# ygina/sidekick

Measured on AMD Instinct MI355X. Metric: quACK encode identifiers/s (device-resident), u32 ids, threshold t=32, higher is better.
Workload: dtype u32; 1 GPU; encode 1e+09 u32 ids per GPU at t=32, device-resident; ids_per_gpu=1000000000, global_ids=1000000000, threshold=32, bits=32, seed=0x5eed0002, parallelism=shard1, collectives=single

## Files before the change

### sidekick_amd/csrc/bsgs.h

```cpp
#pragma once
#include <hip/hip_runtime.h>
#include <stdint.h>

#include "field.h"

namespace qk {
namespace bsgs {

constexpr int BLOCK = 256;
constexpr int WAVES = BLOCK / 64;

__device__ __forceinline__ uint64_t shfl_xor_u64(uint64_t v, int m) {
    const uint32_t lo = __shfl_xor((int)(uint32_t)v, m, 64);
    const uint32_t hi = __shfl_xor((int)(uint32_t)(v >> 32), m, 64);
    return ((uint64_t)hi << 32) | lo;
}

#define QK_MAC4V(P0, P1, P2, P3)                                                                       \
    "v_mad_u64_u32 %0, " P0 ", %8, %9, %0\n\t"                                                         \
    "v_mad_u64_u32 %1, " P1 ", %8, %10, %1\n\t"                                                        \
    "v_mad_u64_u32 %2, " P2 ", %8, %11, %2\n\t"                                                        \
    "v_mad_u64_u32 %3, " P3 ", %8, %12, %3\n\t"                                                        \
    "v_addc_co_u32_e64 %4, " P0 ", %4, 0, " P0 "\n\t"                                                  \
    "v_addc_co_u32_e64 %5, " P1 ", %5, 0, " P1 "\n\t"                                                  \
    "v_addc_co_u32_e64 %6, " P2 ", %6, 0, " P2 "\n\t"                                                  \
    "v_addc_co_u32_e64 %7, " P3 ", %7, 0, " P3
#define QK_MAC4S(P0, P1, P2, P3, T)                                                                       \
    "v_mad_u64_u32 %0, " P0 ", %8, %9, %0\n\t"                                                         \
    "v_mad_u64_u32 %1, " P1 ", %8, %10, %1\n\t"                                                        \
    "v_mad_u64_u32 %2, " P2 ", %8, %11, %2\n\t"                                                        \
    "v_mad_u64_u32 %3, " P3 ", %8, %12, %3\n\t"                                                        \
    "s_bcnt1_i32_b64 " T ", " P0 "\n\ts_add_u32 %4, %4, " T "\n\t"                                          \
    "s_bcnt1_i32_b64 " T ", " P1 "\n\ts_add_u32 %5, %5, " T "\n\t"                                          \
    "s_bcnt1_i32_b64 " T ", " P2 "\n\ts_add_u32 %6, %6, " T "\n\t"                                          \
    "s_bcnt1_i32_b64 " T ", " P3 "\n\ts_add_u32 %7, %7, " T
#define QK_ADD4V(P0, P1, P2, P3)                                                                       \
    "v_add_co_u32_e64 %0, " P0 ", %0, %8\n\t"                                                          \
    "v_add_co_u32_e64 %1, " P1 ", %1, %9\n\t"                                                          \
    "v_add_co_u32_e64 %2, " P2 ", %2, %10\n\t"                                                         \
    "v_add_co_u32_e64 %3, " P3 ", %3, %11\n\t"                                                         \
    "v_addc_co_u32_e64 %4, " P0 ", %4, 0, " P0 "\n\t"                                                  \
    "v_addc_co_u32_e64 %5, " P1 ", %5, 0, " P1 "\n\t"                                                  \
    "v_addc_co_u32_e64 %6, " P2 ", %6, 0, " P2 "\n\t"                                                  \
    "v_addc_co_u32_e64 %7, " P3 ", %7, 0, " P3
#define QK_ADD4S(P0, P1, P2, P3, T)                                                                       \
    "v_add_co_u32_e64 %0, " P0 ", %0, %8\n\t"                                                          \
    "v_add_co_u32_e64 %1, " P1 ", %1, %9\n\t"                                                          \
    "v_add_co_u32_e64 %2, " P2 ", %2, %10\n\t"                                                         \
    "v_add_co_u32_e64 %3, " P3 ", %3, %11\n\t"                                                         \
    "s_bcnt1_i32_b64 " T ", " P0 "\n\ts_add_u32 %4, %4, " T "\n\t"                                          \
    "s_bcnt1_i32_b64 " T ", " P1 "\n\ts_add_u32 %5, %5, " T "\n\t"                                          \
    "s_bcnt1_i32_b64 " T ", " P2 "\n\ts_add_u32 %6, %6, " T "\n\t"                                          \
    "s_bcnt1_i32_b64 " T ", " P3 "\n\ts_add_u32 %7, %7, " T
#define QK_SET0 "s[40:41]", "s[42:43]", "s[44:45]", "s[46:47]"
#define QK_SET1 "s[48:49]", "s[50:51]", "s[52:53]", "s[54:55]"
#define QK_SET0T QK_SET0, "s56"
#define QK_SET1T QK_SET1, "s57"
#define QK_CLOB0 "s40", "s41", "s42", "s43", "s44", "s45", "s46", "s47"
#define QK_CLOB1 "s48", "s49", "s50", "s51", "s52", "s53", "s54", "s55"
#define QK_EXPAND(M, ...) M(__VA_ARGS__)

template <int SET>
__device__ __forceinline__ void mac4v(uint64_t &a0, uint64_t &a1, uint64_t &a2, uint64_t &a3, uint32_t &c0,
                                      uint32_t &c1, uint32_t &c2, uint32_t &c3, uint32_t A, uint32_t b0,
                                      uint32_t b1, uint32_t b2, uint32_t b3) {
    if constexpr (SET == 0)
        asm volatile(QK_EXPAND(QK_MAC4V, QK_SET0)
            : "+v"(a0), "+v"(a1), "+v"(a2), "+v"(a3), "+v"(c0), "+v"(c1), "+v"(c2), "+v"(c3)
            : "v"(A), "v"(b0), "v"(b1), "v"(b2), "v"(b3)
            : QK_CLOB0);
    else
        asm volatile(QK_EXPAND(QK_MAC4V, QK_SET1)
            : "+v"(a0), "+v"(a1), "+v"(a2), "+v"(a3), "+v"(c0), "+v"(c1), "+v"(c2), "+v"(c3)
            : "v"(A), "v"(b0), "v"(b1), "v"(b2), "v"(b3)
            : QK_CLOB1);
}
template <int SET>
__device__ __forceinline__ void mac4s(uint64_t &a0, uint64_t &a1, uint64_t &a2, uint64_t &a3, uint32_t &s0,
                                      uint32_t &s1, uint32_t &s2, uint32_t &s3, uint32_t A, uint32_t b0,
                                      uint32_t b1, uint32_t b2, uint32_t b3) {
    if constexpr (SET == 0)
        asm volatile(QK_EXPAND(QK_MAC4S, QK_SET0T)
            : "+v"(a0), "+v"(a1), "+v"(a2), "+v"(a3), "+s"(s0), "+s"(s1), "+s"(s2), "+s"(s3)
            : "v"(A), "v"(b0), "v"(b1), "v"(b2), "v"(b3)
            : "scc", "s56", QK_CLOB0);
    else
        asm volatile(QK_EXPAND(QK_MAC4S, QK_SET1T)
            : "+v"(a0), "+v"(a1), "+v"(a2), "+v"(a3), "+s"(s0), "+s"(s1), "+s"(s2), "+s"(s3)
            : "v"(A), "v"(b0), "v"(b1), "v"(b2), "v"(b3)
            : "scc", "s57", QK_CLOB1);
}
template <int SET>
__device__ __forceinline__ void add4v(uint32_t &l0, uint32_t &l1, uint32_t &l2, uint32_t &l3, uint32_t &c0,
                                      uint32_t &c1, uint32_t &c2, uint32_t &c3, uint32_t b0, uint32_t b1,
                                      uint32_t b2, uint32_t b3) {
    if constexpr (SET == 0)
        asm volatile(QK_EXPAND(QK_ADD4V, QK_SET0)
            : "+v"(l0), "+v"(l1), "+v"(l2), "+v"(l3), "+v"(c0), "+v"(c1), "+v"(c2), "+v"(c3)
            : "v"(b0), "v"(b1), "v"(b2), "v"(b3)
            : QK_CLOB0);
    else
        asm volatile(QK_EXPAND(QK_ADD4V, QK_SET1)
            : "+v"(l0), "+v"(l1), "+v"(l2), "+v"(l3), "+v"(c0), "+v"(c1), "+v"(c2), "+v"(c3)
            : "v"(b0), "v"(b1), "v"(b2), "v"(b3)
            : QK_CLOB1);
}
template <int SET>
__device__ __forceinline__ void add4s(uint32_t &l0, uint32_t &l1, uint32_t &l2, uint32_t &l3, uint32_t &s0,
                                      uint32_t &s1, uint32_t &s2, uint32_t &s3, uint32_t b0, uint32_t b1,
                                      uint32_t b2, uint32_t b3) {
    if constexpr (SET == 0)
        asm volatile(QK_EXPAND(QK_ADD4S, QK_SET0T)
            : "+v"(l0), "+v"(l1), "+v"(l2), "+v"(l3), "+s"(s0), "+s"(s1), "+s"(s2), "+s"(s3)
            : "v"(b0), "v"(b1), "v"(b2), "v"(b3)
            : "scc", "s56", QK_CLOB0);
    else
        asm volatile(QK_EXPAND(QK_ADD4S, QK_SET1T)
            : "+v"(l0), "+v"(l1), "+v"(l2), "+v"(l3), "+s"(s0), "+s"(s1), "+s"(s2), "+s"(s3)
            : "v"(b0), "v"(b1), "v"(b2), "v"(b3)
            : "scc", "s57", QK_CLOB1);
}
__device__ __forceinline__ void mac2v(uint64_t &a0, uint64_t &a1, uint32_t &c0, uint32_t &c1, uint32_t A,
                                      uint32_t b0, uint32_t b1) {
    uint64_t k0, k1;
    asm("v_mad_u64_u32 %0, %4, %6, %7, %0\n\t"
        "v_mad_u64_u32 %1, %5, %6, %8, %1\n\t"
        "s_nop 0\n\t"
        "v_addc_co_u32_e64 %2, %4, %2, 0, %4\n\t"
        "v_addc_co_u32_e64 %3, %5, %3, 0, %5"
        : "+v"(a0), "+v"(a1), "+v"(c0), "+v"(c1), "=&s"(k0), "=&s"(k1)
        : "v"(A), "v"(b0), "v"(b1));
}
__device__ __forceinline__ void add2v(uint32_t &l0, uint32_t &l1, uint32_t &c0, uint32_t &c1, uint32_t b0,
                                      uint32_t b1) {
    uint64_t k0, k1;
    asm("v_add_co_u32_e64 %0, %4, %0, %6\n\t"
        "v_add_co_u32_e64 %1, %5, %1, %7\n\t"
        "s_nop 0\n\t"
        "v_addc_co_u32_e64 %2, %4, %2, 0, %4\n\t"
        "v_addc_co_u32_e64 %3, %5, %3, 0, %5"
        : "+v"(l0), "+v"(l1), "+v"(c0), "+v"(c1), "=&s"(k0), "=&s"(k1)
        : "v"(b0), "v"(b1));
}

#define QK_ROW4M(P0, P1, P2, P3)                                                                       \
    "v_mad_u64_u32 %0, " P0 ", %4, 1, %0\n\t"                                                          \
    "v_mad_u64_u32 %1, " P1 ", %5, 1, %1\n\t"                                                          \
    "v_mad_u64_u32 %2, " P2 ", %6, 1, %2\n\t"                                                          \
    "v_mad_u64_u32 %3, " P3 ", %7, 1, %3"
template <int SET>
__device__ __forceinline__ void row4m(uint64_t &a0, uint64_t &a1, uint64_t &a2, uint64_t &a3, uint32_t b0,
                                      uint32_t b1, uint32_t b2, uint32_t b3) {
    if constexpr (SET == 0)
        asm volatile(QK_EXPAND(QK_ROW4M, QK_SET0)
            : "+v"(a0), "+v"(a1), "+v"(a2), "+v"(a3)
            : "v"(b0), "v"(b1), "v"(b2), "v"(b3)
            : QK_CLOB0);
    else
        asm volatile(QK_EXPAND(QK_ROW4M, QK_SET1)
            : "+v"(a0), "+v"(a1), "+v"(a2), "+v"(a3)
            : "v"(b0), "v"(b1), "v"(b2), "v"(b3)
            : QK_CLOB1);
}
__device__ __forceinline__ void row2m(uint64_t &a0, uint64_t &a1, uint32_t b0, uint32_t b1) {
    uint64_t k0, k1;
    asm("v_mad_u64_u32 %0, %2, %4, 1, %0\n\t"
        "v_mad_u64_u32 %1, %3, %5, 1, %1"
        : "+v"(a0), "+v"(a1), "=&s"(k0), "=&s"(k1)
        : "v"(b0), "v"(b1));
}

template <int NB_, int NA_, int SG_, int ROW0_ = 1, int FOLD_ = 1, bool PAIR_ = false, bool OFF_ = false,
          int XC_ = 0, bool TREE_ = false, int PRIO_ = 0>
struct Cfg {
    static constexpr int PRIO = PRIO_;
    static constexpr int NB = NB_, NA = NA_, SG = SG_, ROW0 = ROW0_, FOLD = FOLD_, XC = XC_;
    static constexpr bool TREE = TREE_;
    static_assert(!TREE_ || (!OFF_ && FOLD_ == 1), "product-tree babies: plain passes, min-tracked folds");
    static constexpr bool PAIR = PAIR_, OFF = OFF_;
    static_assert(OFF_ || (XC_ & 1) == 0, "only an offset pass reads x^base");
    static_assert(!XC_ || FOLD_ == 1, "the x^base cache goes with min-tracked folds");
    static constexpr int ROWS = OFF_ ? NA_ : NA_ - 1;
    static constexpr int ROW1 = OFF_ ? 0 : 1;
    static_assert(NB % 2 == 0 && (NA >= 2 || (OFF_ && NA == 1)), "NB even, NA >= 2 (1: offset pass)");
    static_assert(!OFF_ || FOLD_ == 1, "offset passes use min-tracked folds");
};

template <int NB, int NA, int ROWS = NA - 1>
struct Acc {
    uint32_t lo0[NB];
    uint32_t c0[NB];
    uint64_t r0[NB];
    uint64_t m[ROWS][NB];
    uint32_t c[ROWS][NB];
};

template <class C>
__host__ __device__ constexpr bool scalar_group(int row, int b) {
    return b / 4 * 4 + 4 <= C::NB && (row > 0 || C::ROW0 == 0 || C::OFF) && row * (C::NB / 4) + b / 4 < C::SG;
}

template <class MUL>
__device__ __forceinline__ uint32_t pow_uniform(uint32_t xn, uint32_t q, MUL mul) {
    uint32_t r = 0, sq = xn;
    bool have = false;
    for (;;) {
        if (q & 1) {
            r = have ? mul(r, sq) : sq;
            have = true;
        }
        q >>= 1;
        if (!q) break;
        sq = mul(sq, sq);
    }
    return r;
}

template <class C>
__device__ __forceinline__ uint32_t powers(uint32_t id, uint32_t (&B)[C::NB], uint32_t (&A)[C::ROWS],
                                           uint32_t base = 0, uint32_t xb = 0, uint32_t *xnext = nullptr) {
    constexpr int NB = C::NB, NA = C::NA;
    B[0] = id;
    if constexpr (C::OFF) {
        uint32_t mn = 0xFFFFFFFFu;
#pragma unroll
        for (int b = 1; b < NB; ++b) B[b] = mulfold32_min(B[b - 1], B[0], mn);
        const uint32_t xn = B[NB - 1];
        if constexpr (C::XC & 1) A[0] = xb;
        else A[0] = pow_uniform(xn, base / NB, [&](uint32_t u, uint32_t v) { return mulfold32_min(u, v, mn); });
#pragma unroll
        for (int a = 1; a < NA; ++a) A[a] = mulfold32_min(A[a - 1], xn, mn);
        if constexpr ((C::XC & 2) != 0) *xnext = mulfold32_min(A[NA - 1], xn, mn);
        return mn < 25u;
    } else if constexpr (C::FOLD == 0) {
        uint32_t wrapped = 0;
#pragma unroll
        for (int b = 1; b < NB; ++b) B[b] = mulfold32_fast(B[b - 1], B[0], wrapped);
        A[0] = B[NB - 1];
#pragma unroll
        for (int a = 1; a < NA - 1; ++a) A[a] = mulfold32_fast(A[a - 1], A[0], wrapped);
        return wrapped;
    } else {
        uint32_t mn = 0xFFFFFFFFu;
        if constexpr (C::TREE) {
#pragma unroll
            for (int b = 1; b < NB; ++b) {
                const int h = 1 << (31 - __builtin_clz((unsigned)(b + 1) - 1u));
                B[b] = (b + 1) == 2 * h ? mulfold32_min(B[h - 1], B[h - 1], mn)
                                        : mulfold32_min(B[h - 1], B[b - h], mn);
            }
        } else {
#pragma unroll
            for (int b = 1; b < NB; ++b) B[b] = mulfold32_min(B[b - 1], B[0], mn);
        }
        A[0] = B[NB - 1];
#pragma unroll
        for (int a = 1; a < NA - 1; ++a) A[a] = mulfold32_min(A[a - 1], A[0], mn);
        if constexpr ((C::XC & 2) != 0) *xnext = mulfold32_min(A[NA - 2], A[0], mn);
        return mn < 25u;
    }
}
template <class C>
__device__ __forceinline__ void powers_exact(uint32_t (&B)[C::NB], uint32_t (&A)[C::ROWS], uint32_t base = 0,
                                             uint32_t xb = 0, uint32_t *xnext = nullptr) {
#pragma unroll
    for (int b = 1; b < C::NB; ++b) B[b] = mulfold32_exact(B[b - 1], B[0]);
    if constexpr (C::OFF) {
        const uint32_t xn = B[C::NB - 1];
        if constexpr (C::XC & 1) A[0] = xb;
        else A[0] = pow_uniform(xn, base / C::NB, [](uint32_t u, uint32_t v) { return mulfold32_exact(u, v); });
#pragma unroll
        for (int a = 1; a < C::NA; ++a) A[a] = mulfold32_exact(A[a - 1], xn);
        if constexpr ((C::XC & 2) != 0) *xnext = mulfold32_exact(A[C::NA - 1], xn);
        return;
    }
    A[0] = B[C::NB - 1];
#pragma unroll
    for (int a = 1; a < C::NA - 1; ++a) A[a] = mulfold32_exact(A[a - 1], A[0]);
    if constexpr ((C::XC & 2) != 0) *xnext = mulfold32_exact(A[C::NA - 2], A[0]);
}

template <class C>
__device__ __forceinline__ void accumulate(Acc<C::NB, C::NA, C::ROWS> &S, const uint32_t (&B)[C::NB],
                                           const uint32_t (&A)[C::ROWS]) {
    constexpr int NB = C::NB;
    auto row0 = [&]() {
    #pragma unroll
        for (int b = 0; b + 4 <= NB; b += 4) {
            if constexpr (C::OFF) break;
            const bool s0 = (b / 4) % 2 == 0;
            if constexpr (C::ROW0 == 1) {
                if (s0) row4m<0>(S.r0[b], S.r0[b + 1], S.r0[b + 2], S.r0[b + 3], B[b], B[b + 1], B[b + 2], B[b + 3]);
                else row4m<1>(S.r0[b], S.r0[b + 1], S.r0[b + 2], S.r0[b + 3], B[b], B[b + 1], B[b + 2], B[b + 3]);
            } else if (scalar_group<C>(0, b)) {
                if (s0)
                    add4s<0>(S.lo0[b], S.lo0[b + 1], S.lo0[b + 2], S.lo0[b + 3], S.c0[b], S.c0[b + 1], S.c0[b + 2],
                             S.c0[b + 3], B[b], B[b + 1], B[b + 2], B[b + 3]);
                else
                    add4s<1>(S.lo0[b], S.lo0[b + 1], S.lo0[b + 2], S.lo0[b + 3], S.c0[b], S.c0[b + 1], S.c0[b + 2],
                             S.c0[b + 3], B[b], B[b + 1], B[b + 2], B[b + 3]);
            } else {
                if (s0)
                    add4v<0>(S.lo0[b], S.lo0[b + 1], S.lo0[b + 2], S.lo0[b + 3], S.c0[b], S.c0[b + 1], S.c0[b + 2],
                             S.c0[b + 3], B[b], B[b + 1], B[b + 2], B[b + 3]);
                else
                    add4v<1>(S.lo0[b], S.lo0[b + 1], S.lo0[b + 2], S.lo0[b + 3], S.c0[b], S.c0[b + 1], S.c0[b + 2],
                             S.c0[b + 3], B[b], B[b + 1], B[b + 2], B[b + 3]);
            }
        }
        if constexpr (NB % 4 == 2 && !C::OFF) {
            if constexpr (C::ROW0 == 1) row2m(S.r0[NB - 2], S.r0[NB - 1], B[NB - 2], B[NB - 1]);
            else add2v(S.lo0[NB - 2], S.lo0[NB - 1], S.c0[NB - 2], S.c0[NB - 1], B[NB - 2], B[NB - 1]);
        }
    };
    if constexpr (C::PRIO != 7) row0();
    if constexpr (C::PRIO == 3) __builtin_amdgcn_s_setprio(1);
    if constexpr (C::PRIO == 4) __builtin_amdgcn_s_setprio(2);
    if constexpr (C::PRIO == 6) __builtin_amdgcn_s_setprio(2);
#pragma unroll
    for (int a = 0; a < C::ROWS; ++a) {
        if constexpr (C::PRIO == 5) {
            if (a == 0) __builtin_amdgcn_s_setprio(2);
            else __builtin_amdgcn_s_setprio(3);
        }
#pragma unroll
        for (int b = 0; b + 4 <= NB; b += 4) {
            const int g = (a + C::ROW1) * (NB / 4) + b / 4;
            if (scalar_group<C>(a + C::ROW1, b)) {
                if (g % 2 == 0)
                    mac4s<0>(S.m[a][b], S.m[a][b + 1], S.m[a][b + 2], S.m[a][b + 3], S.c[a][b], S.c[a][b + 1],
                             S.c[a][b + 2], S.c[a][b + 3], A[a], B[b], B[b + 1], B[b + 2], B[b + 3]);
                else
                    mac4s<1>(S.m[a][b], S.m[a][b + 1], S.m[a][b + 2], S.m[a][b + 3], S.c[a][b], S.c[a][b + 1],
                             S.c[a][b + 2], S.c[a][b + 3], A[a], B[b], B[b + 1], B[b + 2], B[b + 3]);
            } else {
                if (g % 2 == 0)
                    mac4v<0>(S.m[a][b], S.m[a][b + 1], S.m[a][b + 2], S.m[a][b + 3], S.c[a][b], S.c[a][b + 1],
                             S.c[a][b + 2], S.c[a][b + 3], A[a], B[b], B[b + 1], B[b + 2], B[b + 3]);
                else
                    mac4v<1>(S.m[a][b], S.m[a][b + 1], S.m[a][b + 2], S.m[a][b + 3], S.c[a][b], S.c[a][b + 1],
                             S.c[a][b + 2], S.c[a][b + 3], A[a], B[b], B[b + 1], B[b + 2], B[b + 3]);
            }
        }
        if constexpr (NB % 4 == 2)
            mac2v(S.m[a][NB - 2], S.m[a][NB - 1], S.c[a][NB - 2], S.c[a][NB - 1], A[a], B[NB - 2], B[NB - 1]);
    }
    if constexpr (C::PRIO == 7) {
        __builtin_amdgcn_s_setprio(1);
        row0();
    }
}

template <class C> __device__ __forceinline__ void prio_enter() {
    if constexpr (C::PRIO == 1 || C::PRIO == 4 || C::PRIO == 5) __builtin_amdgcn_s_setprio(1);
    if constexpr (C::PRIO == 6) __builtin_amdgcn_s_setprio(3);
    if constexpr (C::PRIO == 7) __builtin_amdgcn_s_setprio(2);
    if constexpr (C::PRIO == 2) __builtin_amdgcn_s_setprio(0);
}
template <class C> __device__ __forceinline__ void prio_exit() {
    if constexpr (C::PRIO == 1 || C::PRIO >= 3) __builtin_amdgcn_s_setprio(0);
    if constexpr (C::PRIO == 2) __builtin_amdgcn_s_setprio(1);
}

template <class C>
__device__ __forceinline__ void one(Acc<C::NB, C::NA, C::ROWS> &S, uint32_t id, uint32_t base = 0, uint32_t xb = 0,
                                    uint32_t *xnext = nullptr) {
    uint32_t B[C::NB], A[C::ROWS];
    const uint32_t w = powers<C>(id, B, A, base, xb, xnext);
    if (__builtin_expect(__any(w), 0)) {
        if (w) powers_exact<C>(B, A, base, xb, xnext);
    }
    prio_enter<C>();
    accumulate<C>(S, B, A);
    prio_exit<C>();
}

template <class C>
__device__ __forceinline__ void two(Acc<C::NB, C::NA, C::ROWS> &S, uint32_t id0, uint32_t id1) {
    static_assert(!C::OFF, "pairs: plain passes only");
    uint32_t B0[C::NB], A0[C::ROWS], B1[C::NB], A1[C::ROWS];
    const uint32_t w0 = powers<C>(id0, B0, A0);
    const uint32_t w1 = powers<C>(id1, B1, A1);
    if (__builtin_expect(__any(w0 | w1), 0)) {
        if (w0) powers_exact<C>(B0, A0);
        if (w1) powers_exact<C>(B1, A1);
    }
    prio_enter<C>();
    accumulate<C>(S, B0, A0);
    accumulate<C>(S, B1, A1);
    prio_exit<C>();
}

template <class C>
__device__ __forceinline__ void four(Acc<C::NB, C::NA, C::ROWS> &S, uint4 w, uint32_t base,
                                     uint4 xb = make_uint4(0, 0, 0, 0), uint4 *xn = nullptr) {
    if constexpr (C::PAIR) {
        two<C>(S, w.x, w.y);
        two<C>(S, w.z, w.w);
    } else {
        uint4 t = make_uint4(0, 0, 0, 0);
        one<C>(S, w.x, base, xb.x, &t.x);
        one<C>(S, w.y, base, xb.y, &t.y);
        one<C>(S, w.z, base, xb.z, &t.z);
        one<C>(S, w.w, base, xb.w, &t.w);
        if constexpr ((C::XC & 2) != 0) *xn = t;
    }
}

template <class C, class Out>
__device__ __forceinline__ void finish(const Acc<C::NB, C::NA, C::ROWS> &S, uint32_t T, Out out) {
    constexpr int NB = C::NB, NA = C::NA;
    __shared__ uint64_t sm[WAVES * NB * NA];
    const int lane = threadIdx.x & 63, wave = threadIdx.x >> 6;
#pragma unroll
    for (int a = 0; a < NA; ++a) {
#pragma unroll
        for (int b = 0; b < NB; ++b) {
            const bool sc = scalar_group<C>(a, b);
            const uint32_t c = C::OFF ? S.c[a][b] : a == 0 ? S.c0[b] : S.c[a - C::ROW1][b];
            const uint32_t cl = sc ? (lane == 0 ? c : 0u) : c;
            uint64_t x;
            if (C::OFF) {
                x = (uint64_t)fold64_32(S.m[a][b]) + fold64_32((uint64_t)cl * 25u);
            } else if (a == 0) {
                if constexpr (C::ROW0 == 1) x = S.r0[b];
                else x = (uint64_t)S.lo0[b] + (uint64_t)cl * 5u;
            } else {
                x = (uint64_t)fold64_32(S.m[a - C::ROW1][b]) + fold64_32((uint64_t)cl * 25u);
            }
            x = fold64_32(x);
#pragma unroll
            for (int off = 32; off >= 1; off >>= 1) x += shfl_xor_u64(x, off);
            if (lane == 0) sm[wave * (NB * NA) + a * NB + b] = x;
        }
    }
    __syncthreads();
    for (uint32_t m = threadIdx.x; m < T; m += BLOCK) {
        uint64_t s = 0;
#pragma unroll
        for (int w = 0; w < WAVES; ++w) s += sm[w * (NB * NA) + m];
        out(m, s);
    }
}

template <class C>
__device__ __forceinline__ void clear(Acc<C::NB, C::NA, C::ROWS> &S) {
#pragma unroll
    for (int b = 0; b < C::NB; ++b) {
        S.lo0[b] = 0;
        S.c0[b] = 0;
        S.r0[b] = 0;
#pragma unroll
        for (int a = 0; a < C::ROWS; ++a) { S.m[a][b] = 0; S.c[a][b] = 0; }
    }
}

template <class C, class Out>
__device__ __forceinline__ void body_gen(const uint32_t *__restrict__ ids, uint64_t n, uint32_t head, uint32_t T,
                                         uint64_t gtid, uint64_t nthr, Out out, uint32_t base = 0,
                                         const uint32_t *xin = nullptr,
                                         uint32_t *xout = nullptr) {
    constexpr bool XI = (C::XC & 1) != 0, XO = (C::XC & 2) != 0;
    Acc<C::NB, C::NA, C::ROWS> S;
    clear<C>(S);
    const uint64_t h = head < n ? head : n;
    const uint64_t nbody = (n - h) >> 2;
    const uint4 *__restrict__ v = reinterpret_cast<const uint4 *>(ids + h);
    const uint32_t iters = gtid < nbody ? (uint32_t)((nbody - gtid + nthr - 1) / nthr) : 0u;
    const uint32_t tmax = (uint32_t)__builtin_amdgcn_readfirstlane(iters);
    const uint32_t tmin = (uint32_t)__builtin_amdgcn_readlane((int)iters, 63);
    const uint4 *__restrict__ p = v + gtid;
    const uint4 *pc = XI ? reinterpret_cast<const uint4 *>(xin + h) + gtid : nullptr;
    uint4 *po = XO ? reinterpret_cast<uint4 *>(xout + h) + gtid : nullptr;
    uint4 nxt = make_uint4(0, 0, 0, 0), nxc = make_uint4(0, 0, 0, 0), xo = make_uint4(0, 0, 0, 0);
    if (iters) {
        nxt = *p;
        if constexpr (XI) nxc = *pc;
    }
    uint32_t it = 0;
    for (; it + 1 < tmin; ++it) {
        const uint4 w = nxt, c = nxc;
        p += nthr;
        nxt = *p;
        if constexpr (XI) {
            pc += nthr;
            nxc = *pc;
        }
        four<C>(S, w, base, c, &xo);
        if constexpr (XO) {
            *po = xo;
            po += nthr;
        }
    }
    for (; it < tmax; ++it) {
        const uint4 w = nxt, c = nxc;
        p += nthr;
        nxt = make_uint4(0, 0, 0, 0);
        if (it + 1 < iters) nxt = *p;
        if constexpr (XI) {
            pc += nthr;
            if (it + 1 < iters) nxc = *pc;
        }
        four<C>(S, w, base, c, &xo);
        if constexpr (XO) {
            if (it < iters) *po = xo;
            po += nthr;
        }
    }
    const uint64_t tail0 = h + (nbody << 2);
    {
        const bool in = gtid < h;
        uint32_t xn = 0;
        one<C>(S, in ? ids[gtid] : 0u, base, XI && in ? xin[gtid] : 0u, &xn);
        if (XO && in) xout[gtid] = xn;
    }
    {
        const bool in = gtid < n - tail0;
        uint32_t xn = 0;
        one<C>(S, in ? ids[tail0 + gtid] : 0u, base, XI && in ? xin[tail0 + gtid] : 0u, &xn);
        if (XO && in) xout[tail0 + gtid] = xn;
    }

    finish<C>(S, T, out);
}

template <class C>
__device__ __forceinline__ void body(const uint32_t *__restrict__ ids, uint64_t n, uint32_t head, uint32_t T,
                                     uint64_t *__restrict__ partials, uint32_t base = 0,
                                     const uint32_t *xin = nullptr, uint32_t *xout = nullptr) {
    body_gen<C>(
        ids, n, head, T, (uint64_t)blockIdx.x * BLOCK + threadIdx.x, (uint64_t)gridDim.x * BLOCK,
        [=](uint32_t m, uint64_t s) { partials[(size_t)m * gridDim.x + blockIdx.x] = s; }, base, xin, xout);
}

}
}
```

### sidekick_amd/csrc/field.h

```cpp
#pragma once
#include <stdint.h>

#if defined(__HIPCC__)
#define QK_HD __host__ __device__ __forceinline__
#else
#define QK_HD static inline
#endif

namespace qk {

constexpr uint32_t P32 = 4294967291u;
constexpr uint64_t P64 = 18446744073709551557ull;
constexpr uint32_t C32 = 5u;
constexpr uint64_t C64 = 59u;

QK_HD uint32_t canon32(uint32_t x) {
    uint32_t a = x + C32;
    return a < x ? a : x;
}

QK_HD uint32_t mul32_lazy(uint32_t y, uint32_t x) {
    uint64_t P = (uint64_t)y * x;
    uint64_t t = (P >> 32) * C32 + (uint32_t)P;
    uint64_t u = (t >> 32) * C32 + (uint32_t)t;
    return (uint32_t)u + C32 * (uint32_t)(u >> 32);
}

QK_HD uint32_t mad32_lazy(uint32_t y, uint32_t x, uint32_t c) {
    uint64_t P = (uint64_t)y * x + c;
    uint64_t t = (P >> 32) * C32 + (uint32_t)P;
    uint64_t u = (t >> 32) * C32 + (uint32_t)t;
    return (uint32_t)u + C32 * (uint32_t)(u >> 32);
}

QK_HD void tstep32(uint32_t &lo, uint32_t &hi, uint32_t x, uint32_t x5, uint32_t c) {
    const uint64_t P = (uint64_t)lo * x + ((uint64_t)hi * x5 + c);
    const uint32_t Ph = (uint32_t)(P >> 32);
    const uint64_t Q = P + (uint64_t)Ph * C32;
    lo = (uint32_t)Q;
    hi = (uint32_t)(Q >> 32) - Ph;
}
QK_HD uint64_t tstep32p(uint64_t t, uint32_t x, uint32_t x5, uint32_t c) {
    const uint64_t P = (uint64_t)(uint32_t)t * x + ((uint64_t)(uint32_t)(t >> 32) * x5 + c);
    const uint32_t Ph = (uint32_t)(P >> 32);
    const uint64_t Q = P + (uint64_t)Ph * C32;
    return Q - ((uint64_t)Ph << 32);
}
QK_HD uint32_t mulfold32_fast(uint32_t y, uint32_t x, uint32_t &wrapped) {
    const uint64_t P = (uint64_t)y * x;
    const uint32_t Ph = (uint32_t)(P >> 32);
    const uint64_t Q = P + (uint64_t)Ph * C32;
    const uint32_t tl = (uint32_t)Q, th = (uint32_t)(Q >> 32) - Ph;
    const uint32_t m = th * C32;
    const uint32_t r = tl + m;
    wrapped |= (r < m);
    return r;
}
QK_HD uint32_t mulfold32_exact(uint32_t y, uint32_t x) {
    const uint64_t P = (uint64_t)y * x;
    const uint32_t Ph = (uint32_t)(P >> 32);
    const uint64_t Q = P + (uint64_t)Ph * C32;
    const uint32_t tl = (uint32_t)Q, th = (uint32_t)(Q >> 32) - Ph;
    const uint32_t m = th * C32;
    uint32_t r = tl + m;
    if (r < m) r += C32;
    return r;
}

QK_HD uint32_t mulfold32_min(uint32_t y, uint32_t x, uint32_t &mn) {
    const uint64_t P = (uint64_t)y * x;
    const uint32_t Ph = (uint32_t)(P >> 32);
    const uint64_t Q = P + (uint64_t)Ph * C32;
    const uint32_t tl = (uint32_t)Q, th = (uint32_t)(Q >> 32) - Ph;
    const uint32_t r = tl + th * C32;
    mn = r < mn ? r : mn;
    return r;
}

QK_HD uint32_t times5_32(uint32_t x) {
    const uint64_t v = (uint64_t)x * C32;
    const uint64_t u = (v >> 32) * C32 + (uint32_t)v;
    const uint32_t r = (uint32_t)u + C32 * (uint32_t)(u >> 32);
    const uint32_t a = r + C32;
    return a < r ? a : r;
}

QK_HD uint32_t fold64_32(uint64_t a) {
    uint64_t t = (a >> 32) * C32 + (uint32_t)a;
    uint64_t u = (t >> 32) * C32 + (uint32_t)t;
    return (uint32_t)u + C32 * (uint32_t)(u >> 32);
}

QK_HD uint32_t add32(uint32_t a, uint32_t b) {
    uint64_t s = (uint64_t)a + b;
    return (uint32_t)(s >= P32 ? s - P32 : s);
}
QK_HD uint32_t sub32(uint32_t a, uint32_t b) {
    return a >= b ? a - b : (uint32_t)((uint64_t)a + P32 - b);
}
QK_HD uint32_t mul32(uint32_t a, uint32_t b) { return canon32(mul32_lazy(a, b)); }
QK_HD uint32_t neg32(uint32_t a) { return a == 0 ? 0 : P32 - a; }
QK_HD uint32_t pow32(uint32_t a, uint64_t e) {
    uint32_t r = 1;
    while (e) {
        if (e & 1) r = mul32(r, a);
        a = mul32(a, a);
        e >>= 1;
    }
    return r;
}
QK_HD uint32_t inv32(uint32_t a) { return pow32(a, P32 - 2); }

QK_HD uint64_t canon64(uint64_t x) {
    uint64_t a = x + C64;
    return a < x ? a : x;
}

QK_HD void mul64_wide(uint64_t a, uint64_t b, uint64_t &hi, uint64_t &lo) {
    unsigned __int128 P = (unsigned __int128)a * b;
    hi = (uint64_t)(P >> 64);
    lo = (uint64_t)P;
}

QK_HD uint64_t mul64_lazy(uint64_t a, uint64_t b) {
    uint64_t H, L;
    mul64_wide(a, b, H, L);
    unsigned __int128 t = (unsigned __int128)H * C64 + L;
    uint64_t th = (uint64_t)(t >> 64), tl = (uint64_t)t;
    unsigned __int128 u = (unsigned __int128)th * C64 + tl;
    return (uint64_t)u + C64 * (uint64_t)(u >> 64);
}

QK_HD uint64_t mad64_lazy(uint64_t a, uint64_t b, uint64_t c) {
    unsigned __int128 P = (unsigned __int128)a * b + c;
    uint64_t H = (uint64_t)(P >> 64), L = (uint64_t)P;
    unsigned __int128 t = (unsigned __int128)H * C64 + L;
    uint64_t th = (uint64_t)(t >> 64), tl = (uint64_t)t;
    unsigned __int128 u = (unsigned __int128)th * C64 + tl;
    return (uint64_t)u + C64 * (uint64_t)(u >> 64);
}

QK_HD void tstep64(uint32_t &t0, uint32_t &t1, uint32_t &th, uint32_t x0, uint32_t x1, uint32_t y0, uint32_t y1) {
    const uint64_t c0 = (uint64_t)t0 * x0;
    const uint64_t c1 = (uint64_t)t1 * x0 + (c0 >> 32);
    const uint64_t c2 = (uint64_t)t0 * x1 + (uint32_t)c1;
    const uint64_t c3 = (uint64_t)t1 * x1 + (c1 >> 32) + (c2 >> 32);
    const uint64_t d0 = (uint64_t)th * y0 + (uint32_t)c0;
    const uint64_t d1 = (uint64_t)th * y1 + (uint32_t)c2 + (d0 >> 32);
    const uint64_t PH = c3 + (d1 >> 32);
    const uint64_t e0 = (uint64_t)(uint32_t)PH * C64 + (uint32_t)d0;
    const uint64_t e1 = (uint64_t)(uint32_t)(PH >> 32) * C64 + (uint32_t)d1 + (e0 >> 32);
    t0 = (uint32_t)e0;
    t1 = (uint32_t)e1;
    th = (uint32_t)(e1 >> 32);
}

QK_HD uint64_t fold96_64(uint32_t hi, uint64_t lo) {
    unsigned __int128 t = (unsigned __int128)hi * C64 + lo;
    uint64_t th = (uint64_t)(t >> 64), tl = (uint64_t)t;
    unsigned __int128 u = (unsigned __int128)th * C64 + tl;
    return (uint64_t)u + C64 * (uint64_t)(u >> 64);
}

QK_HD uint64_t add64(uint64_t a, uint64_t b) {
    uint64_t s = a + b;
    if (s < a) return s + C64;
    return s >= P64 ? s - P64 : s;
}
QK_HD uint64_t sub64(uint64_t a, uint64_t b) {
    return a >= b ? a - b : a + (P64 - b);
}
QK_HD uint64_t mul64(uint64_t a, uint64_t b) { return canon64(mul64_lazy(a, b)); }
QK_HD uint64_t neg64(uint64_t a) { return a == 0 ? 0 : P64 - a; }
QK_HD uint64_t pow64(uint64_t a, uint64_t e) {
    uint64_t r = 1;
    while (e) {
        if (e & 1) r = mul64(r, a);
        a = mul64(a, a);
        e >>= 1;
    }
    return r;
}
QK_HD uint64_t inv64(uint64_t a) { return pow64(a, P64 - 2); }

constexpr uint64_t GAMMA = 0x9E3779B97F4A7C15ull;
QK_HD uint64_t splitmix_mix(uint64_t z) {
    z = (z ^ (z >> 30)) * 0xBF58476D1CE4E5B9ull;
    z = (z ^ (z >> 27)) * 0x94D049BB133111EBull;
    return z ^ (z >> 31);
}

}
```

### sidekick_amd/csrc/packets.hip

```cpp
#include <string.h>

#include <algorithm>
#include <type_traits>
#include <vector>

#include "bsgs.h"
#include "ctx.h"
#include "field.h"
#include "records.h"

namespace qk {

QK_WARM_KERNEL(packets)

constexpr int PK_BLOCK = REC_TILE;
constexpr uint64_t PK_WGPC = 4;

struct ChunkStat {
    int64_t last_reset;
    int64_t last_insert;
    uint64_t inserts;
    uint64_t resets;
    uint64_t all_inserts;
    uint64_t last_insert_id;
};

struct NoEncode {};
template <int NA_> struct Shared {
    static constexpr int NA = NA_;
    using Pw = bsgs::Cfg<8, NA_, 0, 1, 1>;
};
template <class C> struct IsShared : std::false_type {};
template <int NA> struct IsShared<Shared<NA>> : std::true_type {};
template <class C, bool SH = IsShared<C>::value> struct AccOf { using type = bsgs::Acc<C::NB, C::NA, C::ROWS>; };
template <class C> struct AccOf<C, true> { using type = int; };
template <> struct AccOf<NoEncode, false> { using type = int; };
template <class C, bool SH = IsShared<C>::value> struct ShNA { static constexpr int value = 1; };
template <class C> struct ShNA<C, true> { static constexpr int value = C::NA; };
template <class C, bool NT = false>
__global__ __launch_bounds__(PK_BLOCK) void k_pkt_kernel(const uint8_t *__restrict__ bufs, uint64_t n,
                                                         uint32_t stride, const qk_pkt_meta *__restrict__ meta,
                                                         uint32_t my_ip_le, int check_reset, uint64_t chunk,
                                                         uint32_t *__restrict__ ids_out, ChunkStat *stats,
                                                         uint32_t T, uint64_t *__restrict__ partials) {
    constexpr bool SH = IsShared<C>::value;
    constexpr bool FUSED = !std::is_same<C, NoEncode>::value && !SH;
    constexpr int SNA = ShNA<C>::value;
    extern __shared__ __attribute__((aligned(16))) uint8_t tile[];
    __shared__ uint32_t sh_v[SH ? 8 + SNA - 2 : 1][SH ? PK_BLOCK : 1];
    [[maybe_unused]] uint64_t sh_acc[SNA][2];
    [[maybe_unused]] uint32_t sh_c[SNA][2];
    if constexpr (SH) {
#pragma unroll
        for (int a = 0; a < SNA; ++a) sh_acc[a][0] = sh_acc[a][1] = 0, sh_c[a][0] = sh_c[a][1] = 0;
    }
    __shared__ int64_t s_reset[PK_BLOCK / 64], s_insert[PK_BLOCK / 64];
    __shared__ uint64_t s_cnt[PK_BLOCK / 64], s_nres[PK_BLOCK / 64], s_nins[PK_BLOCK / 64], s_iid[PK_BLOCK / 64];
    [[maybe_unused]] typename AccOf<C>::type S;
    if constexpr (FUSED) bsgs::clear<C>(S);
    uint64_t blk_iid = 0;
    const uint64_t c0 = (uint64_t)blockIdx.x * chunk;
    const uint64_t c1 = c0 + chunk < n ? c0 + chunk : n;
    const int lane = threadIdx.x & 63, wave = threadIdx.x >> 6;

    int64_t blk_reset = -1;
    uint64_t blk_cnt = 0;
    int64_t blk_insert = -1;
    uint64_t blk_nres = 0, blk_nins = 0;

    const bool pipe = stage_pipelined(stride, PK_BLOCK);
    TileStage st;
    if (pipe && c0 < c1) stage_issue<NT>(bufs, n, stride, c0, c1 - c0 < PK_BLOCK ? c1 - c0 : PK_BLOCK, st);
    for (uint64_t p0 = c0; p0 < c1; p0 += PK_BLOCK) {
        const uint64_t np = (c1 - p0) < PK_BLOCK ? (c1 - p0) : PK_BLOCK;
        __syncthreads();
        const uint32_t r0 = pipe ? stage_commit(bufs, n, stride, st, tile) : stage_records<NT>(bufs, n, stride, p0, np, tile);
        __syncthreads();
        if (pipe && p0 + PK_BLOCK < c1)
            stage_issue<NT>(bufs, n, stride, p0 + PK_BLOCK, c1 - p0 - PK_BLOCK < PK_BLOCK ? c1 - p0 - PK_BLOCK : PK_BLOCK, st);
        uint32_t cls = 0, id = 0;
        const uint64_t pi = p0 + threadIdx.x;
        if (threadIdx.x < np) {
            const uint8_t *rec = tile + r0 + threadIdx.x * stride;
            const qk_pkt_meta m = record_meta<NT>(meta, pi);
            if (record_is_incoming_udp(m, rec)) {
                const uint32_t dst = (uint32_t)rec[30] | ((uint32_t)rec[31] << 8) | ((uint32_t)rec[32] << 16) |
                                     ((uint32_t)rec[33] << 24);
                if (check_reset && dst == my_ip_le) cls = 2;
                else if (m.len == (uint32_t)QK_BUFFER_SIZE) {
                    cls = 1;
                    id = record_identifier(rec);
                }
            }
            if constexpr (std::is_same<C, NoEncode>::value) ids_out[pi] = cls == 1 ? id : 0u;
        }
        if constexpr (FUSED) bsgs::one<C>(S, cls == 1 ? id : 0u);
        if constexpr (SH) {
            using Pw = typename C::Pw;
            uint32_t B[8], A[Pw::ROWS];
            const uint32_t w = bsgs::powers<Pw>(cls == 1 ? id : 0u, B, A);
            if (__builtin_expect(__any(w), 0)) {
                if (w) bsgs::powers_exact<Pw>(B, A);
            }
#pragma unroll
            for (int b = 0; b < 8; ++b) sh_v[b][threadIdx.x] = B[b];
#pragma unroll
            for (int r = 1; r < Pw::ROWS; ++r) sh_v[7 + r][threadIdx.x] = A[r];
        }
        const unsigned long long rmask = __ballot(cls == 2);
        const unsigned long long imask = __ballot(cls == 1);
        const uint32_t last_id = (uint32_t)__shfl((int)id, imask ? 63 - __clzll(imask) : 0, 64);
        if (lane == 0) {
            int64_t wr = -1, wi = -1;
            uint64_t wc;
            if (rmask) {
                const int hb = 63 - __clzll(rmask);
                wr = (int64_t)(p0 + wave * 64 + hb);
                const unsigned long long after = hb == 63 ? 0ull : (imask & (~0ull << (hb + 1)));
                wc = __popcll(after);
            } else {
                wc = __popcll(imask);
            }
            if (imask) wi = (int64_t)(p0 + wave * 64 + 63 - __clzll(imask));
            s_reset[wave] = wr;
            s_iid[wave] = 0;
            s_insert[wave] = wi;
            s_cnt[wave] = wc;
            s_nres[wave] = __popcll(rmask);
            s_nins[wave] = __popcll(imask);
            s_iid[wave] = last_id;
        }
        __syncthreads();
        if constexpr (SH) {
            const int b0 = 2 * wave;
#pragma unroll
            for (int q = 0; q < PK_BLOCK / 64; ++q) {
                const int j = q * 64 + lane;
                const uint32_t B0 = sh_v[b0][j], B1 = sh_v[b0 + 1][j];
                bsgs::row2m(sh_acc[0][0], sh_acc[0][1], B0, B1);
#pragma unroll
                for (int a = 1; a < SNA; ++a)
                    bsgs::mac2v(sh_acc[a][0], sh_acc[a][1], sh_c[a][0], sh_c[a][1], sh_v[6 + a][j], B0, B1);
            }
        }
        if (threadIdx.x == 0) {
            for (int w = 0; w < PK_BLOCK / 64; ++w) {
                blk_nres += s_nres[w];
                blk_nins += s_nins[w];
                if (s_reset[w] >= 0) { blk_reset = s_reset[w]; blk_cnt = s_cnt[w]; blk_insert = -1; }
                else blk_cnt += s_cnt[w];
                if (s_insert[w] > blk_reset && s_insert[w] > blk_insert) {
                    blk_insert = s_insert[w];
                    blk_iid = s_iid[w];
                }
            }
        }
    }
    if (threadIdx.x == 0) {
        ChunkStat st;
        st.last_reset = blk_reset;
        st.last_insert = blk_insert;
        st.inserts = blk_cnt;
        st.resets = blk_nres;
        st.all_inserts = blk_nins;
        st.last_insert_id = blk_iid;
        stats[blockIdx.x] = st;
    }
    if constexpr (FUSED)
        bsgs::finish<C>(S, T, [=](uint32_t m, uint64_t v) { partials[(size_t)m * gridDim.x + blockIdx.x] = v; });
    if constexpr (SH) {
#pragma unroll
        for (int a = 0; a < SNA; ++a) {
#pragma unroll
            for (int k = 0; k < 2; ++k) {
                const uint32_t m = 8 * a + 2 * wave + k;
                uint64_t x = a == 0 ? fold64_32(sh_acc[0][k])
                                    : (uint64_t)fold64_32(sh_acc[a][k]) + fold64_32((uint64_t)sh_c[a][k] * 25u);
                x = fold64_32(x);
#pragma unroll
                for (int off = 32; off >= 1; off >>= 1) x += bsgs::shfl_xor_u64(x, off);
                if (lane == 0 && m < T) partials[(size_t)m * gridDim.x + blockIdx.x] = x;
            }
        }
    }
}

}

using namespace qk;

extern "C" int qk_u32_encode_packets_device(qk_ctx *ctx, const uint8_t *d_bufs, size_t n, size_t stride,
                                            const qk_pkt_meta *d_meta, const uint8_t my_ipv4[4], qk_u32 *q,
                                            qk_pkt_stats *out_stats, void *stream) {
    if (!ctx || !q || (n && !d_bufs)) return QK_E_INVAL;
    if (stride < QK_BUFFER_SIZE || stride > 512) return QK_E_INVAL;
    const uint32_t t = q->threshold;
    if (t == 0 || t > QK_MAX_THRESHOLD) return QK_E_THRESHOLD;
    qk_pkt_stats st = {0, 0, 0, 0, -1};
    if (n == 0) {
        if (out_stats) *out_stats = st;
        return QK_OK;
    }
    if (!is_device_ptr(d_bufs) || (d_meta && !is_device_ptr(d_meta))) return QK_E_INVAL;
    const uint32_t my_ip_le = my_ipv4 ? ((uint32_t)my_ipv4[0] | ((uint32_t)my_ipv4[1] << 8) |
                                         ((uint32_t)my_ipv4[2] << 16) | ((uint32_t)my_ipv4[3] << 24))
                                      : 0u;
    const int check_reset = my_ipv4 != nullptr;
    std::lock_guard<std::mutex> g(ctx->mu);
    QK_HIP_TRY(hipSetDevice(ctx->device));
    hipStream_t s = pick_stream(ctx, stream);

    const uint64_t tiles = (n + PK_BLOCK - 1) / PK_BLOCK;
    const uint64_t wgs = (uint64_t)ctx->num_cus * PK_WGPC;
    uint64_t tiles_per_chunk = std::max<uint64_t>(4, (tiles + wgs - 1) / wgs);
    const uint64_t chunk = tiles_per_chunk * PK_BLOCK;
    const uint32_t nchunks = (uint32_t)((n + chunk - 1) / chunk);

    const size_t ids_bytes = ((size_t)n * sizeof(uint32_t) + 255) & ~(size_t)255;
    if (int e = ensure_flow(ctx, 0, ids_bytes + (size_t)nchunks * sizeof(ChunkStat), s)) return e;
    uint32_t *d_ids = (uint32_t *)ctx->d_flow[0];
    ChunkStat *d_stats = (ChunkStat *)((char *)ctx->d_flow[0] + ids_bytes);
    const size_t lds = (size_t)PK_BLOCK * stride + 32;
    int rc = QK_OK;
    std::vector<ChunkStat> hs(nchunks);
    if (t >= 5 && t <= 32) {
        int frc = QK_OK;
        if (int e = ensure_scratch(ctx, (size_t)nchunks * 32 * sizeof(uint64_t), s)) return e;
        if (int e = scratch_acquire(ctx, s)) return e;
        uint64_t *partials = (uint64_t *)ctx->d_scratch;
#define QK_PKT_FUSED(NB_, NA_, SG_)                                                                          \
    hipLaunchKernelGGL((k_pkt_kernel<bsgs::Cfg<NB_, NA_, SG_>, true>), dim3(nchunks), dim3(PK_BLOCK), lds, s, d_bufs,                                                \
                       (uint64_t)n, (uint32_t)stride, d_meta, my_ip_le, check_reset, chunk, (uint32_t *)nullptr,   \
                       d_stats, t, partials)
        hipEvent_t e0 = prof_begin(ctx, s);
        if (t <= 8) QK_PKT_FUSED(4, 2, 0);
        else if (t <= 12) QK_PKT_FUSED(4, 3, 0);
#undef QK_PKT_FUSED
#define QK_PKT_SHARED(NA_)                                                                                       \
    hipLaunchKernelGGL((k_pkt_kernel<Shared<NA_>, true>), dim3(nchunks), dim3(PK_BLOCK), lds, s, d_bufs, (uint64_t)n, \
                       (uint32_t)stride, d_meta, my_ip_le, check_reset, chunk, (uint32_t *)nullptr, d_stats, t,         \
                       partials)
        else if (t <= 16) QK_PKT_SHARED(2);
        else if (t <= 24) QK_PKT_SHARED(3);
        else QK_PKT_SHARED(4);
#undef QK_PKT_SHARED
        prof_end(ctx, s, e0);
        if (hipGetLastError() != hipSuccess) frc = QK_E_HIP;
        if (!frc) frc = launch_finalize_powers_u32(partials, nchunks, t, ctx->d_small, s);
        if (int e = scratch_release(ctx, s); e && !frc) frc = e;
        if (!frc && (hipMemcpyAsync(hs.data(), d_stats, nchunks * sizeof(ChunkStat), hipMemcpyDeviceToHost, s) !=
                         hipSuccess ||
                     hipMemcpyAsync(ctx->h_small, ctx->d_small, (size_t)t * 8, hipMemcpyDeviceToHost, s) != hipSuccess ||
                     hipStreamSynchronize(s) != hipSuccess))
            frc = QK_E_HIP;
        if (frc) return frc;
        uint64_t resets = 0, inserts = 0;
        int64_t last_insert = -1;
        uint32_t last_id = 0;
        for (const ChunkStat &c : hs) {
            resets += c.resets;
            inserts += c.inserts;
            if (c.last_insert > last_insert) { last_insert = c.last_insert; last_id = (uint32_t)c.last_insert_id; }
        }
        if (resets == 0) {
            st.inserted = inserts;
            st.filtered = n - inserts;
            qk_u32 *tmp = (qk_u32 *)malloc(qk_u32_size(t));
            if (!tmp) return QK_E_NOMEM;
            qk_u32_init(tmp, t);
            ctx->h_small[t] = inserts;
            rc = qk_u32_merge_partial(tmp, ctx->h_small, last_insert >= 0, last_id);
            if (!rc) rc = qk_u32_merge(q, tmp);
            free(tmp);
            if (out_stats) *out_stats = st;
            return rc;
        }
    }
    auto kx = k_pkt_kernel<NoEncode, true>;
    hipLaunchKernelGGL(kx, dim3(nchunks), dim3(PK_BLOCK), lds, s, d_bufs, (uint64_t)n,
                       (uint32_t)stride, d_meta, my_ip_le, check_reset, chunk, d_ids, d_stats, 0u,
                       (uint64_t *)nullptr);
    if (hipGetLastError() != hipSuccess) rc = QK_E_HIP;
    if (!rc && hipMemcpyAsync(hs.data(), d_stats, nchunks * sizeof(ChunkStat), hipMemcpyDeviceToHost, s) != hipSuccess)
        rc = QK_E_HIP;
    if (!rc && hipStreamSynchronize(s) != hipSuccess) rc = QK_E_HIP;
    if (!rc) {
        int64_t last_reset = -1, last_insert = -1;
        uint64_t inserts = 0, resets = 0, all_inserts = 0;
        for (const ChunkStat &c : hs) {
            resets += c.resets;
            all_inserts += c.all_inserts;
            if (c.last_reset >= 0) { last_reset = c.last_reset; inserts = c.inserts; last_insert = -1; }
            else inserts += c.inserts;
            if (c.last_insert > last_reset && c.last_insert > last_insert) last_insert = c.last_insert;
        }
        st.resets = resets;
        st.last_reset_index = last_reset;
        st.inserted = inserts;
        st.discarded = all_inserts - inserts;
        const uint64_t from = (uint64_t)(last_reset + 1);
        qk_u32 *tmp = (qk_u32 *)malloc(qk_u32_size(t));
        if (!tmp) rc = QK_E_NOMEM;
        else {
            qk_u32_init(tmp, t);
            if (from < n) rc = launch_encode_u32(ctx, d_ids + from, n - from, t, ctx->d_small, s);
            if (!rc && from < n) {
                const size_t w = qk_u32_partial_words(t);
                uint32_t last_id = 0;
                if (hipMemcpyAsync(ctx->h_small, ctx->d_small, w * 8, hipMemcpyDeviceToHost, s) != hipSuccess ||
                    (last_insert >= 0 &&
                     hipMemcpyAsync(&last_id, d_ids + last_insert, 4, hipMemcpyDeviceToHost, s) != hipSuccess) ||
                    hipStreamSynchronize(s) != hipSuccess)
                    rc = QK_E_HIP;
                else {
                    ctx->h_small[t] = inserts;
                    rc = qk_u32_merge_partial(tmp, ctx->h_small, last_insert >= 0, last_id);
                }
            }
            if (!rc) {
                if (last_reset >= 0) qk_u32_init(q, t);
                rc = qk_u32_merge(q, tmp);
            }
            free(tmp);
        }
    }
    (void)hipStreamSynchronize(s);
    st.filtered = n - st.inserted - st.discarded - st.resets;
    if (out_stats) *out_stats = st;
    return rc;
}
```

Before: 408.2 billion identifiers/s.

## Fuse lazy power chains in inline asm and defer wrap check past priority boost

Adds a fused inline-asm lazy product chain (LazyChain) that computes the baby-step and giant-step powers with two v_mad_u64_u32 fold steps each, and rewrites mulfold32_min in asm with hard-coded registers. powers now returns the running minimum, and the wrap test moves after prio_enter with a sched_barrier so the accumulation priority window covers it. The main loop bounds by pointer comparison, and the thread index is rematerialized from scalar registers after the loop to ease register pressure. Hard-coded v6/v7/s58/s59 clobbers in asm are fragile and may conflict with compiler allocation.

Measured after the change: 447.2 billion identifiers/s, median of 6. +9.5%, better.

```diff
diff --git a/profiles/lazy_product/main_loop_branch.s b/profiles/lazy_product/main_loop_branch.s
--- /dev/null
+++ b/profiles/lazy_product/main_loop_branch.s
@@ -0,0 +1,506 @@
+.LBB53_10:
+	v_lshl_add_u64 v[6:7], v[92:93], 0, s[24:25]
+	global_load_dwordx4 v[14:17], v[6:7], off offset:-8
+	s_waitcnt vmcnt(1)
+	v_mad_u64_u32 v[38:39], s[58:59], v0, v0, 0
+	v_mad_u64_u32 v[6:7], s[58:59], v39, 5, v[38:39]
+	v_mad_u64_u32 v[38:39], s[58:59], v7, 5, v[38:39]
+	v_mad_u64_u32 v[36:37], s[58:59], v38, v0, 0
+	v_mad_u64_u32 v[6:7], s[58:59], v37, 5, v[36:37]
+	v_mad_u64_u32 v[36:37], s[58:59], v7, 5, v[36:37]
+	v_mad_u64_u32 v[34:35], s[58:59], v36, v0, 0
+	v_mad_u64_u32 v[6:7], s[58:59], v35, 5, v[34:35]
+	v_mad_u64_u32 v[34:35], s[58:59], v7, 5, v[34:35]
+	v_mad_u64_u32 v[32:33], s[58:59], v34, v0, 0
+	v_mad_u64_u32 v[6:7], s[58:59], v33, 5, v[32:33]
+	v_mad_u64_u32 v[32:33], s[58:59], v7, 5, v[32:33]
+	v_mad_u64_u32 v[30:31], s[58:59], v32, v0, 0
+	v_mad_u64_u32 v[6:7], s[58:59], v31, 5, v[30:31]
+	v_mad_u64_u32 v[30:31], s[58:59], v7, 5, v[30:31]
+	v_mad_u64_u32 v[28:29], s[58:59], v30, v0, 0
+	v_mad_u64_u32 v[6:7], s[58:59], v29, 5, v[28:29]
+	v_mad_u64_u32 v[28:29], s[58:59], v7, 5, v[28:29]
+	v_mad_u64_u32 v[8:9], s[58:59], v28, v0, 0
+	v_mad_u64_u32 v[6:7], s[58:59], v9, 5, v[8:9]
+	v_mad_u64_u32 v[8:9], s[58:59], v7, 5, v[8:9]
+	v_mad_u64_u32 v[10:11], s[58:59], v8, v8, 0
+	v_mad_u64_u32 v[6:7], s[58:59], v11, 5, v[10:11]
+	v_mad_u64_u32 v[10:11], s[58:59], v7, 5, v[10:11]
+	v_mad_u64_u32 v[12:13], s[58:59], v10, v8, 0
+	v_mad_u64_u32 v[6:7], s[58:59], v13, 5, v[12:13]
+	v_mad_u64_u32 v[12:13], s[58:59], v7, 5, v[12:13]
+	v_min3_u32 v9, v30, v28, v8
+	v_min3_u32 v9, v9, v34, v32
+	v_min3_u32 v9, v9, v38, v36
+	v_min3_u32 v9, v9, v10, v12
+	
+	s_setprio 1
+	v_cmp_gt_u32_e32 vcc, 25, v9
+	s_cbranch_vccnz .LBB53_16
+.LBB53_11:
+	v_mad_u64_u32 v[90:91], s[40:41], v0, 1, v[90:91]
+	v_mad_u64_u32 v[88:89], s[42:43], v38, 1, v[88:89]
+	v_mad_u64_u32 v[86:87], s[44:45], v36, 1, v[86:87]
+	v_mad_u64_u32 v[84:85], s[46:47], v34, 1, v[84:85]
+	v_mad_u64_u32 v[82:83], s[48:49], v32, 1, v[82:83]
+	v_mad_u64_u32 v[80:81], s[50:51], v30, 1, v[80:81]
+	v_mad_u64_u32 v[78:79], s[52:53], v28, 1, v[78:79]
+	v_mad_u64_u32 v[76:77], s[54:55], v8, 1, v[76:77]
+	s_setprio 2
+	v_mad_u64_u32 v[74:75], s[40:41], v8, v0, v[74:75]
+	v_mad_u64_u32 v[72:73], s[42:43], v8, v38, v[72:73]
+	v_mad_u64_u32 v[70:71], s[44:45], v8, v36, v[70:71]
+	v_mad_u64_u32 v[68:69], s[46:47], v8, v34, v[68:69]
+	s_bcnt1_i32_b64 s56, s[40:41]
+	s_add_u32 s72, s72, s56
+	s_bcnt1_i32_b64 s56, s[42:43]
+	s_add_u32 s71, s71, s56
+	s_bcnt1_i32_b64 s56, s[44:45]
+	s_add_u32 s70, s70, s56
+	s_bcnt1_i32_b64 s56, s[46:47]
+	s_add_u32 s69, s69, s56
+	s_nop 0
+	v_mad_u64_u32 v[66:67], s[48:49], v8, v32, v[66:67]
+	v_mad_u64_u32 v[64:65], s[50:51], v8, v30, v[64:65]
+	v_mad_u64_u32 v[62:63], s[52:53], v8, v28, v[62:63]
+	v_mad_u64_u32 v[60:61], s[54:55], v8, v8, v[60:61]
+	s_bcnt1_i32_b64 s57, s[48:49]
+	s_add_u32 s68, s68, s57
+	s_bcnt1_i32_b64 s57, s[50:51]
+	s_add_u32 s67, s67, s57
+	s_bcnt1_i32_b64 s57, s[52:53]
+	s_add_u32 s66, s66, s57
+	s_bcnt1_i32_b64 s57, s[54:55]
+	s_add_u32 s65, s65, s57
+	s_nop 0
+	v_mad_u64_u32 v[58:59], s[40:41], v10, v0, v[58:59]
+	v_mad_u64_u32 v[56:57], s[42:43], v10, v38, v[56:57]
+	v_mad_u64_u32 v[54:55], s[44:45], v10, v36, v[54:55]
+	v_mad_u64_u32 v[52:53], s[46:47], v10, v34, v[52:53]
+	s_bcnt1_i32_b64 s56, s[40:41]
+	s_add_u32 s64, s64, s56
+	s_bcnt1_i32_b64 s56, s[42:43]
+	s_add_u32 s63, s63, s56
+	s_bcnt1_i32_b64 s56, s[44:45]
+	s_add_u32 s62, s62, s56
+	s_bcnt1_i32_b64 s56, s[46:47]
+	s_add_u32 s61, s61, s56
+	s_nop 0
+	v_mad_u64_u32 v[50:51], s[48:49], v10, v32, v[50:51]
+	v_mad_u64_u32 v[48:49], s[50:51], v10, v30, v[48:49]
+	v_mad_u64_u32 v[46:47], s[52:53], v10, v28, v[46:47]
+	v_mad_u64_u32 v[44:45], s[54:55], v10, v8, v[44:45]
+	s_bcnt1_i32_b64 s57, s[48:49]
+	s_add_u32 s60, s60, s57
+	s_bcnt1_i32_b64 s57, s[50:51]
+	s_add_u32 s39, s39, s57
+	s_bcnt1_i32_b64 s57, s[52:53]
+	s_add_u32 s38, s38, s57
+	s_bcnt1_i32_b64 s57, s[54:55]
+	s_add_u32 s37, s37, s57
+	s_nop 0
+	v_mad_u64_u32 v[42:43], s[40:41], v12, v0, v[42:43]
+	v_mad_u64_u32 v[40:41], s[42:43], v12, v38, v[40:41]
+	v_mad_u64_u32 v[26:27], s[44:45], v12, v36, v[26:27]
+	v_mad_u64_u32 v[24:25], s[46:47], v12, v34, v[24:25]
+	s_bcnt1_i32_b64 s56, s[40:41]
+	s_add_u32 s36, s36, s56
+	s_bcnt1_i32_b64 s56, s[42:43]
+	s_add_u32 s35, s35, s56
+	s_bcnt1_i32_b64 s56, s[44:45]
+	s_add_u32 s34, s34, s56
+	s_bcnt1_i32_b64 s56, s[46:47]
+	s_add_u32 s33, s33, s56
+	s_nop 0
+	v_mad_u64_u32 v[22:23], s[48:49], v12, v32, v[22:23]
+	v_mad_u64_u32 v[20:21], s[50:51], v12, v30, v[20:21]
+	v_mad_u64_u32 v[18:19], s[52:53], v12, v28, v[18:19]
+	v_mad_u64_u32 v[4:5], s[54:55], v12, v8, v[4:5]
+	s_bcnt1_i32_b64 s57, s[48:49]
+	s_add_u32 s31, s31, s57
+	s_bcnt1_i32_b64 s57, s[50:51]
+	s_add_u32 s29, s29, s57
+	s_bcnt1_i32_b64 s57, s[52:53]
+	s_add_u32 s28, s28, s57
+	s_bcnt1_i32_b64 s57, s[54:55]
+	s_add_u32 s12, s12, s57
+	s_setprio 0
+	v_mad_u64_u32 v[38:39], s[58:59], v1, v1, 0
+	v_mad_u64_u32 v[6:7], s[58:59], v39, 5, v[38:39]
+	v_mad_u64_u32 v[38:39], s[58:59], v7, 5, v[38:39]
+	v_mad_u64_u32 v[36:37], s[58:59], v38, v1, 0
+	v_mad_u64_u32 v[6:7], s[58:59], v37, 5, v[36:37]
+	v_mad_u64_u32 v[36:37], s[58:59], v7, 5, v[36:37]
+	v_mad_u64_u32 v[34:35], s[58:59], v36, v1, 0
+	v_mad_u64_u32 v[6:7], s[58:59], v35, 5, v[34:35]
+	v_mad_u64_u32 v[34:35], s[58:59], v7, 5, v[34:35]
+	v_mad_u64_u32 v[32:33], s[58:59], v34, v1, 0
+	v_mad_u64_u32 v[6:7], s[58:59], v33, 5, v[32:33]
+	v_mad_u64_u32 v[32:33], s[58:59], v7, 5, v[32:33]
+	v_mad_u64_u32 v[30:31], s[58:59], v32, v1, 0
+	v_mad_u64_u32 v[6:7], s[58:59], v31, 5, v[30:31]
+	v_mad_u64_u32 v[30:31], s[58:59], v7, 5, v[30:31]
+	v_mad_u64_u32 v[28:29], s[58:59], v30, v1, 0
+	v_mad_u64_u32 v[6:7], s[58:59], v29, 5, v[28:29]
+	v_mad_u64_u32 v[28:29], s[58:59], v7, 5, v[28:29]
+	v_mad_u64_u32 v[8:9], s[58:59], v28, v1, 0
+	v_mad_u64_u32 v[6:7], s[58:59], v9, 5, v[8:9]
+	v_mad_u64_u32 v[8:9], s[58:59], v7, 5, v[8:9]
+	v_mad_u64_u32 v[10:11], s[58:59], v8, v8, 0
+	v_mad_u64_u32 v[6:7], s[58:59], v11, 5, v[10:11]
+	v_mad_u64_u32 v[10:11], s[58:59], v7, 5, v[10:11]
+	v_mad_u64_u32 v[12:13], s[58:59], v10, v8, 0
+	v_mad_u64_u32 v[6:7], s[58:59], v13, 5, v[12:13]
+	v_mad_u64_u32 v[12:13], s[58:59], v7, 5, v[12:13]
+	v_min3_u32 v9, v30, v28, v8
+	v_min3_u32 v9, v9, v34, v32
+	v_min3_u32 v9, v9, v38, v36
+	v_min3_u32 v9, v9, v10, v12
+	
+	s_setprio 1
+	v_cmp_gt_u32_e32 vcc, 25, v9
+	s_cbranch_vccnz .LBB53_19
+.LBB53_12:
+	v_mad_u64_u32 v[90:91], s[40:41], v1, 1, v[90:91]
+	v_mad_u64_u32 v[88:89], s[42:43], v38, 1, v[88:89]
+	v_mad_u64_u32 v[86:87], s[44:45], v36, 1, v[86:87]
+	v_mad_u64_u32 v[84:85], s[46:47], v34, 1, v[84:85]
+	v_mad_u64_u32 v[82:83], s[48:49], v32, 1, v[82:83]
+	v_mad_u64_u32 v[80:81], s[50:51], v30, 1, v[80:81]
+	v_mad_u64_u32 v[78:79], s[52:53], v28, 1, v[78:79]
+	v_mad_u64_u32 v[76:77], s[54:55], v8, 1, v[76:77]
+	s_setprio 2
+	v_mad_u64_u32 v[74:75], s[40:41], v8, v1, v[74:75]
+	v_mad_u64_u32 v[72:73], s[42:43], v8, v38, v[72:73]
+	v_mad_u64_u32 v[70:71], s[44:45], v8, v36, v[70:71]
+	v_mad_u64_u32 v[68:69], s[46:47], v8, v34, v[68:69]
+	s_bcnt1_i32_b64 s56, s[40:41]
+	s_add_u32 s72, s72, s56
+	s_bcnt1_i32_b64 s56, s[42:43]
+	s_add_u32 s71, s71, s56
+	s_bcnt1_i32_b64 s56, s[44:45]
+	s_add_u32 s70, s70, s56
+	s_bcnt1_i32_b64 s56, s[46:47]
+	s_add_u32 s69, s69, s56
+	s_nop 0
+	v_mad_u64_u32 v[66:67], s[48:49], v8, v32, v[66:67]
+	v_mad_u64_u32 v[64:65], s[50:51], v8, v30, v[64:65]
+	v_mad_u64_u32 v[62:63], s[52:53], v8, v28, v[62:63]
+	v_mad_u64_u32 v[60:61], s[54:55], v8, v8, v[60:61]
+	s_bcnt1_i32_b64 s57, s[48:49]
+	s_add_u32 s68, s68, s57
+	s_bcnt1_i32_b64 s57, s[50:51]
+	s_add_u32 s67, s67, s57
+	s_bcnt1_i32_b64 s57, s[52:53]
+	s_add_u32 s66, s66, s57
+	s_bcnt1_i32_b64 s57, s[54:55]
+	s_add_u32 s65, s65, s57
+	s_nop 0
+	v_mad_u64_u32 v[58:59], s[40:41], v10, v1, v[58:59]
+	v_mad_u64_u32 v[56:57], s[42:43], v10, v38, v[56:57]
+	v_mad_u64_u32 v[54:55], s[44:45], v10, v36, v[54:55]
+	v_mad_u64_u32 v[52:53], s[46:47], v10, v34, v[52:53]
+	s_bcnt1_i32_b64 s56, s[40:41]
+	s_add_u32 s64, s64, s56
+	s_bcnt1_i32_b64 s56, s[42:43]
+	s_add_u32 s63, s63, s56
+	s_bcnt1_i32_b64 s56, s[44:45]
+	s_add_u32 s62, s62, s56
+	s_bcnt1_i32_b64 s56, s[46:47]
+	s_add_u32 s61, s61, s56
+	s_nop 0
+	v_mad_u64_u32 v[50:51], s[48:49], v10, v32, v[50:51]
+	v_mad_u64_u32 v[48:49], s[50:51], v10, v30, v[48:49]
+	v_mad_u64_u32 v[46:47], s[52:53], v10, v28, v[46:47]
+	v_mad_u64_u32 v[44:45], s[54:55], v10, v8, v[44:45]
+	s_bcnt1_i32_b64 s57, s[48:49]
+	s_add_u32 s60, s60, s57
+	s_bcnt1_i32_b64 s57, s[50:51]
+	s_add_u32 s39, s39, s57
+	s_bcnt1_i32_b64 s57, s[52:53]
+	s_add_u32 s38, s38, s57
+	s_bcnt1_i32_b64 s57, s[54:55]
+	s_add_u32 s37, s37, s57
+	s_nop 0
+	v_mad_u64_u32 v[42:43], s[40:41], v12, v1, v[42:43]
+	v_mad_u64_u32 v[40:41], s[42:43], v12, v38, v[40:41]
+	v_mad_u64_u32 v[26:27], s[44:45], v12, v36, v[26:27]
+	v_mad_u64_u32 v[24:25], s[46:47], v12, v34, v[24:25]
+	s_bcnt1_i32_b64 s56, s[40:41]
+	s_add_u32 s36, s36, s56
+	s_bcnt1_i32_b64 s56, s[42:43]
+	s_add_u32 s35, s35, s56
+	s_bcnt1_i32_b64 s56, s[44:45]
+	s_add_u32 s34, s34, s56
+	s_bcnt1_i32_b64 s56, s[46:47]
+	s_add_u32 s33, s33, s56
+	s_nop 0
+	v_mad_u64_u32 v[22:23], s[48:49], v12, v32, v[22:23]
+	v_mad_u64_u32 v[20:21], s[50:51], v12, v30, v[20:21]
+	v_mad_u64_u32 v[18:19], s[52:53], v12, v28, v[18:19]
+	v_mad_u64_u32 v[4:5], s[54:55], v12, v8, v[4:5]
+	s_bcnt1_i32_b64 s57, s[48:49]
+	s_add_u32 s31, s31, s57
+	s_bcnt1_i32_b64 s57, s[50:51]
+	s_add_u32 s29, s29, s57
+	s_bcnt1_i32_b64 s57, s[52:53]
+	s_add_u32 s28, s28, s57
+	s_bcnt1_i32_b64 s57, s[54:55]
+	s_add_u32 s12, s12, s57
+	s_setprio 0
+	v_mad_u64_u32 v[38:39], s[58:59], v2, v2, 0
+	v_mad_u64_u32 v[6:7], s[58:59], v39, 5, v[38:39]
+	v_mad_u64_u32 v[38:39], s[58:59], v7, 5, v[38:39]
+	v_mad_u64_u32 v[36:37], s[58:59], v38, v2, 0
+	v_mad_u64_u32 v[6:7], s[58:59], v37, 5, v[36:37]
+	v_mad_u64_u32 v[36:37], s[58:59], v7, 5, v[36:37]
+	v_mad_u64_u32 v[34:35], s[58:59], v36, v2, 0
+	v_mad_u64_u32 v[6:7], s[58:59], v35, 5, v[34:35]
+	v_mad_u64_u32 v[34:35], s[58:59], v7, 5, v[34:35]
+	v_mad_u64_u32 v[32:33], s[58:59], v34, v2, 0
+	v_mad_u64_u32 v[6:7], s[58:59], v33, 5, v[32:33]
+	v_mad_u64_u32 v[32:33], s[58:59], v7, 5, v[32:33]
+	v_mad_u64_u32 v[30:31], s[58:59], v32, v2, 0
+	v_mad_u64_u32 v[6:7], s[58:59], v31, 5, v[30:31]
+	v_mad_u64_u32 v[30:31], s[58:59], v7, 5, v[30:31]
+	v_mad_u64_u32 v[28:29], s[58:59], v30, v2, 0
+	v_mad_u64_u32 v[6:7], s[58:59], v29, 5, v[28:29]
+	v_mad_u64_u32 v[28:29], s[58:59], v7, 5, v[28:29]
+	v_mad_u64_u32 v[8:9], s[58:59], v28, v2, 0
+	v_mad_u64_u32 v[6:7], s[58:59], v9, 5, v[8:9]
+	v_mad_u64_u32 v[8:9], s[58:59], v7, 5, v[8:9]
+	v_mad_u64_u32 v[10:11], s[58:59], v8, v8, 0
+	v_mad_u64_u32 v[6:7], s[58:59], v11, 5, v[10:11]
+	v_mad_u64_u32 v[10:11], s[58:59], v7, 5, v[10:11]
+	v_mad_u64_u32 v[12:13], s[58:59], v10, v8, 0
+	v_mad_u64_u32 v[6:7], s[58:59], v13, 5, v[12:13]
+	v_mad_u64_u32 v[12:13], s[58:59], v7, 5, v[12:13]
+	v_min3_u32 v9, v30, v28, v8
+	v_min3_u32 v9, v9, v34, v32
+	v_min3_u32 v9, v9, v38, v36
+	v_min3_u32 v9, v9, v10, v12
+	
+	s_setprio 1
+	v_cmp_gt_u32_e32 vcc, 25, v9
+	s_cbranch_vccnz .LBB53_22
+.LBB53_13:
+	v_mad_u64_u32 v[90:91], s[40:41], v2, 1, v[90:91]
+	v_mad_u64_u32 v[88:89], s[42:43], v38, 1, v[88:89]
+	v_mad_u64_u32 v[86:87], s[44:45], v36, 1, v[86:87]
+	v_mad_u64_u32 v[84:85], s[46:47], v34, 1, v[84:85]
+	v_mad_u64_u32 v[82:83], s[48:49], v32, 1, v[82:83]
+	v_mad_u64_u32 v[80:81], s[50:51], v30, 1, v[80:81]
+	v_mad_u64_u32 v[78:79], s[52:53], v28, 1, v[78:79]
+	v_mad_u64_u32 v[76:77], s[54:55], v8, 1, v[76:77]
+	s_setprio 2
+	v_mad_u64_u32 v[74:75], s[40:41], v8, v2, v[74:75]
+	v_mad_u64_u32 v[72:73], s[42:43], v8, v38, v[72:73]
+	v_mad_u64_u32 v[70:71], s[44:45], v8, v36, v[70:71]
+	v_mad_u64_u32 v[68:69], s[46:47], v8, v34, v[68:69]
+	s_bcnt1_i32_b64 s56, s[40:41]
+	s_add_u32 s72, s72, s56
+	s_bcnt1_i32_b64 s56, s[42:43]
+	s_add_u32 s71, s71, s56
+	s_bcnt1_i32_b64 s56, s[44:45]
+	s_add_u32 s70, s70, s56
+	s_bcnt1_i32_b64 s56, s[46:47]
+	s_add_u32 s69, s69, s56
+	s_nop 0
+	v_mad_u64_u32 v[66:67], s[48:49], v8, v32, v[66:67]
+	v_mad_u64_u32 v[64:65], s[50:51], v8, v30, v[64:65]
+	v_mad_u64_u32 v[62:63], s[52:53], v8, v28, v[62:63]
+	v_mad_u64_u32 v[60:61], s[54:55], v8, v8, v[60:61]
+	s_bcnt1_i32_b64 s57, s[48:49]
+	s_add_u32 s68, s68, s57
+	s_bcnt1_i32_b64 s57, s[50:51]
+	s_add_u32 s67, s67, s57
+	s_bcnt1_i32_b64 s57, s[52:53]
+	s_add_u32 s66, s66, s57
+	s_bcnt1_i32_b64 s57, s[54:55]
+	s_add_u32 s65, s65, s57
+	s_nop 0
+	v_mad_u64_u32 v[58:59], s[40:41], v10, v2, v[58:59]
+	v_mad_u64_u32 v[56:57], s[42:43], v10, v38, v[56:57]
+	v_mad_u64_u32 v[54:55], s[44:45], v10, v36, v[54:55]
+	v_mad_u64_u32 v[52:53], s[46:47], v10, v34, v[52:53]
+	s_bcnt1_i32_b64 s56, s[40:41]
+	s_add_u32 s64, s64, s56
+	s_bcnt1_i32_b64 s56, s[42:43]
+	s_add_u32 s63, s63, s56
+	s_bcnt1_i32_b64 s56, s[44:45]
+	s_add_u32 s62, s62, s56
+	s_bcnt1_i32_b64 s56, s[46:47]
+	s_add_u32 s61, s61, s56
+	s_nop 0
+	v_mad_u64_u32 v[50:51], s[48:49], v10, v32, v[50:51]
+	v_mad_u64_u32 v[48:49], s[50:51], v10, v30, v[48:49]
+	v_mad_u64_u32 v[46:47], s[52:53], v10, v28, v[46:47]
+	v_mad_u64_u32 v[44:45], s[54:55], v10, v8, v[44:45]
+	s_bcnt1_i32_b64 s57, s[48:49]
+	s_add_u32 s60, s60, s57
+	s_bcnt1_i32_b64 s57, s[50:51]
+	s_add_u32 s39, s39, s57
+	s_bcnt1_i32_b64 s57, s[52:53]
+	s_add_u32 s38, s38, s57
+	s_bcnt1_i32_b64 s57, s[54:55]
+	s_add_u32 s37, s37, s57
+	s_nop 0
+	v_mad_u64_u32 v[42:43], s[40:41], v12, v2, v[42:43]
+	v_mad_u64_u32 v[40:41], s[42:43], v12, v38, v[40:41]
+	v_mad_u64_u32 v[26:27], s[44:45], v12, v36, v[26:27]
+	v_mad_u64_u32 v[24:25], s[46:47], v12, v34, v[24:25]
+	s_bcnt1_i32_b64 s56, s[40:41]
+	s_add_u32 s36, s36, s56
+	s_bcnt1_i32_b64 s56, s[42:43]
+	s_add_u32 s35, s35, s56
+	s_bcnt1_i32_b64 s56, s[44:45]
+	s_add_u32 s34, s34, s56
+	s_bcnt1_i32_b64 s56, s[46:47]
+	s_add_u32 s33, s33, s56
+	s_nop 0
+	v_mad_u64_u32 v[22:23], s[48:49], v12, v32, v[22:23]
+	v_mad_u64_u32 v[20:21], s[50:51], v12, v30, v[20:21]
+	v_mad_u64_u32 v[18:19], s[52:53], v12, v28, v[18:19]
+	v_mad_u64_u32 v[4:5], s[54:55], v12, v8, v[4:5]
+	s_bcnt1_i32_b64 s57, s[48:49]
+	s_add_u32 s31, s31, s57
+	s_bcnt1_i32_b64 s57, s[50:51]
+	s_add_u32 s29, s29, s57
+	s_bcnt1_i32_b64 s57, s[52:53]
+	s_add_u32 s28, s28, s57
+	s_bcnt1_i32_b64 s57, s[54:55]
+	s_add_u32 s12, s12, s57
+	s_setprio 0
+	v_mad_u64_u32 v[38:39], s[58:59], v3, v3, 0
+	v_mad_u64_u32 v[6:7], s[58:59], v39, 5, v[38:39]
+	v_mad_u64_u32 v[38:39], s[58:59], v7, 5, v[38:39]
+	v_mad_u64_u32 v[36:37], s[58:59], v38, v3, 0
+	v_mad_u64_u32 v[6:7], s[58:59], v37, 5, v[36:37]
+	v_mad_u64_u32 v[36:37], s[58:59], v7, 5, v[36:37]
+	v_mad_u64_u32 v[34:35], s[58:59], v36, v3, 0
+	v_mad_u64_u32 v[6:7], s[58:59], v35, 5, v[34:35]
+	v_mad_u64_u32 v[34:35], s[58:59], v7, 5, v[34:35]
+	v_mad_u64_u32 v[32:33], s[58:59], v34, v3, 0
+	v_mad_u64_u32 v[6:7], s[58:59], v33, 5, v[32:33]
+	v_mad_u64_u32 v[32:33], s[58:59], v7, 5, v[32:33]
+	v_mad_u64_u32 v[30:31], s[58:59], v32, v3, 0
+	v_mad_u64_u32 v[6:7], s[58:59], v31, 5, v[30:31]
+	v_mad_u64_u32 v[30:31], s[58:59], v7, 5, v[30:31]
+	v_mad_u64_u32 v[28:29], s[58:59], v30, v3, 0
+	v_mad_u64_u32 v[6:7], s[58:59], v29, 5, v[28:29]
+	v_mad_u64_u32 v[28:29], s[58:59], v7, 5, v[28:29]
+	v_mad_u64_u32 v[8:9], s[58:59], v28, v3, 0
+	v_mad_u64_u32 v[6:7], s[58:59], v9, 5, v[8:9]
+	v_mad_u64_u32 v[8:9], s[58:59], v7, 5, v[8:9]
+	v_mad_u64_u32 v[10:11], s[58:59], v8, v8, 0
+	v_mad_u64_u32 v[6:7], s[58:59], v11, 5, v[10:11]
+	v_mad_u64_u32 v[10:11], s[58:59], v7, 5, v[10:11]
+	v_mad_u64_u32 v[12:13], s[58:59], v10, v8, 0
+	v_mad_u64_u32 v[6:7], s[58:59], v13, 5, v[12:13]
+	v_mad_u64_u32 v[12:13], s[58:59], v7, 5, v[12:13]
+	v_min3_u32 v9, v30, v28, v8
+	v_min3_u32 v9, v9, v34, v32
+	v_min3_u32 v9, v9, v38, v36
+	v_min3_u32 v9, v9, v10, v12
+	
+	s_setprio 1
+	v_cmp_gt_u32_e32 vcc, 25, v9
+	s_cbranch_vccnz .LBB53_25
+.LBB53_14:
+	v_mad_u64_u32 v[90:91], s[40:41], v3, 1, v[90:91]
+	v_mad_u64_u32 v[88:89], s[42:43], v38, 1, v[88:89]
+	v_mad_u64_u32 v[86:87], s[44:45], v36, 1, v[86:87]
+	v_mad_u64_u32 v[84:85], s[46:47], v34, 1, v[84:85]
+	v_mad_u64_u32 v[82:83], s[48:49], v32, 1, v[82:83]
+	v_mad_u64_u32 v[80:81], s[50:51], v30, 1, v[80:81]
+	v_mad_u64_u32 v[78:79], s[52:53], v28, 1, v[78:79]
+	v_mad_u64_u32 v[76:77], s[54:55], v8, 1, v[76:77]
+	s_setprio 2
+	v_mad_u64_u32 v[74:75], s[40:41], v8, v3, v[74:75]
+	v_mad_u64_u32 v[72:73], s[42:43], v8, v38, v[72:73]
+	v_mad_u64_u32 v[70:71], s[44:45], v8, v36, v[70:71]
+	v_mad_u64_u32 v[68:69], s[46:47], v8, v34, v[68:69]
+	s_bcnt1_i32_b64 s56, s[40:41]
+	s_add_u32 s72, s72, s56
+	s_bcnt1_i32_b64 s56, s[42:43]
+	s_add_u32 s71, s71, s56
+	s_bcnt1_i32_b64 s56, s[44:45]
+	s_add_u32 s70, s70, s56
+	s_bcnt1_i32_b64 s56, s[46:47]
+	s_add_u32 s69, s69, s56
+	s_nop 0
+	v_mad_u64_u32 v[66:67], s[48:49], v8, v32, v[66:67]
+	v_mad_u64_u32 v[64:65], s[50:51], v8, v30, v[64:65]
+	v_mad_u64_u32 v[62:63], s[52:53], v8, v28, v[62:63]
+	v_mad_u64_u32 v[60:61], s[54:55], v8, v8, v[60:61]
+	s_bcnt1_i32_b64 s57, s[48:49]
+	s_add_u32 s68, s68, s57
+	s_bcnt1_i32_b64 s57, s[50:51]
+	s_add_u32 s67, s67, s57
+	s_bcnt1_i32_b64 s57, s[52:53]
+	s_add_u32 s66, s66, s57
+	s_bcnt1_i32_b64 s57, s[54:55]
+	s_add_u32 s65, s65, s57
+	s_nop 0
+	v_mad_u64_u32 v[58:59], s[40:41], v10, v3, v[58:59]
+	v_mad_u64_u32 v[56:57], s[42:43], v10, v38, v[56:57]
+	v_mad_u64_u32 v[54:55], s[44:45], v10, v36, v[54:55]
+	v_mad_u64_u32 v[52:53], s[46:47], v10, v34, v[52:53]
+	s_bcnt1_i32_b64 s56, s[40:41]
+	s_add_u32 s64, s64, s56
+	s_bcnt1_i32_b64 s56, s[42:43]
+	s_add_u32 s63, s63, s56
+	s_bcnt1_i32_b64 s56, s[44:45]
+	s_add_u32 s62, s62, s56
+	s_bcnt1_i32_b64 s56, s[46:47]
+	s_add_u32 s61, s61, s56
+	s_nop 0
+	v_mad_u64_u32 v[50:51], s[48:49], v10, v32, v[50:51]
+	v_mad_u64_u32 v[48:49], s[50:51], v10, v30, v[48:49]
+	v_mad_u64_u32 v[46:47], s[52:53], v10, v28, v[46:47]
+	v_mad_u64_u32 v[44:45], s[54:55], v10, v8, v[44:45]
+	s_bcnt1_i32_b64 s57, s[48:49]
+	s_add_u32 s60, s60, s57
+	s_bcnt1_i32_b64 s57, s[50:51]
+	s_add_u32 s39, s39, s57
+	s_bcnt1_i32_b64 s57, s[52:53]
+	s_add_u32 s38, s38, s57
+	s_bcnt1_i32_b64 s57, s[54:55]
+	s_add_u32 s37, s37, s57
+	s_nop 0
+	v_mad_u64_u32 v[42:43], s[40:41], v12, v3, v[42:43]
+	v_mad_u64_u32 v[40:41], s[42:43], v12, v38, v[40:41]
+	v_mad_u64_u32 v[26:27], s[44:45], v12, v36, v[26:27]
+	v_mad_u64_u32 v[24:25], s[46:47], v12, v34, v[24:25]
+	s_bcnt1_i32_b64 s56, s[40:41]
+	s_add_u32 s36, s36, s56
+	s_bcnt1_i32_b64 s56, s[42:43]
+	s_add_u32 s35, s35, s56
+	s_bcnt1_i32_b64 s56, s[44:45]
+	s_add_u32 s34, s34, s56
+	s_bcnt1_i32_b64 s56, s[46:47]
+	s_add_u32 s33, s33, s56
+	s_nop 0
+	v_mad_u64_u32 v[22:23], s[48:49], v12, v32, v[22:23]
+	v_mad_u64_u32 v[20:21], s[50:51], v12, v30, v[20:21]
+	v_mad_u64_u32 v[18:19], s[52:53], v12, v28, v[18:19]
+	v_mad_u64_u32 v[4:5], s[54:55], v12, v8, v[4:5]
+	s_bcnt1_i32_b64 s57, s[48:49]
+	s_add_u32 s31, s31, s57
+	s_bcnt1_i32_b64 s57, s[50:51]
+	s_add_u32 s29, s29, s57
+	s_bcnt1_i32_b64 s57, s[52:53]
+	s_add_u32 s28, s28, s57
+	s_bcnt1_i32_b64 s57, s[54:55]
+	s_add_u32 s12, s12, s57
+	s_setprio 0
+	s_add_i32 s75, s75, -1
+	s_cmp_eq_u32 s75, 0
+	v_lshl_add_u64 v[92:93], v[92:93], 0, s[0:1]
+	s_cbranch_scc1 .LBB53_29
+	s_waitcnt vmcnt(0)
+	v_mov_b32_e32 v3, v17
+	v_mov_b32_e32 v2, v16
+	v_mov_b32_e32 v1, v15
+	v_mov_b32_e32 v0, v14
+	s_branch .LBB53_10
diff --git a/profiles/lazy_product/main_loop_parent.s b/profiles/lazy_product/main_loop_parent.s
--- /dev/null
+++ b/profiles/lazy_product/main_loop_parent.s
@@ -0,0 +1,542 @@
+.LBB53_10:
+	v_lshl_add_u64 v[6:7], v[78:79], 0, s[20:21]
+	global_load_dwordx4 v[6:9], v[6:7], off offset:-8
+	s_waitcnt vmcnt(2)
+	v_mad_u64_u32 v[74:75], s[22:23], v2, v2, 0
+	v_mad_u64_u32 v[80:81], s[22:23], v75, 5, v[74:75]
+	v_sub_u32_e32 v1, v81, v75
+	v_lshl_add_u32 v77, v1, 2, v1
+	v_add_u32_e32 v1, v77, v80
+	v_mad_u64_u32 v[74:75], s[22:23], v1, v2, 0
+	v_mad_u64_u32 v[80:81], s[22:23], v75, 5, v[74:75]
+	v_sub_u32_e32 v74, v81, v75
+	v_mad_u64_u32 v[80:81], s[22:23], v74, 5, v[80:81]
+	v_mad_u64_u32 v[74:75], s[22:23], v80, v2, 0
+	v_mad_u64_u32 v[82:83], s[22:23], v75, 5, v[74:75]
+	v_sub_u32_e32 v74, v83, v75
+	v_mad_u64_u32 v[82:83], s[22:23], v74, 5, v[82:83]
+	v_mad_u64_u32 v[74:75], s[22:23], v82, v2, 0
+	v_mad_u64_u32 v[84:85], s[22:23], v75, 5, v[74:75]
+	v_sub_u32_e32 v74, v85, v75
+	v_mad_u64_u32 v[84:85], s[22:23], v74, 5, v[84:85]
+	v_mad_u64_u32 v[74:75], s[22:23], v84, v2, 0
+	v_mad_u64_u32 v[86:87], s[22:23], v75, 5, v[74:75]
+	v_sub_u32_e32 v74, v87, v75
+	v_mad_u64_u32 v[86:87], s[22:23], v74, 5, v[86:87]
+	v_mad_u64_u32 v[74:75], s[22:23], v86, v2, 0
+	v_mad_u64_u32 v[88:89], s[22:23], v75, 5, v[74:75]
+	v_sub_u32_e32 v74, v89, v75
+	v_mad_u64_u32 v[88:89], s[22:23], v74, 5, v[88:89]
+	v_mad_u64_u32 v[74:75], s[22:23], v88, v2, 0
+	v_mad_u64_u32 v[90:91], s[22:23], v75, 5, v[74:75]
+	v_sub_u32_e32 v74, v91, v75
+	v_mad_u64_u32 v[90:91], s[22:23], v74, 5, v[90:91]
+	v_mad_u64_u32 v[74:75], s[22:23], v90, v90, 0
+	v_mad_u64_u32 v[92:93], s[22:23], v75, 5, v[74:75]
+	v_sub_u32_e32 v74, v93, v75
+	v_mad_u64_u32 v[92:93], s[22:23], v74, 5, v[92:93]
+	v_mad_u64_u32 v[74:75], s[22:23], v92, v90, 0
+	v_min3_u32 v81, v82, v80, v1
+	v_mad_u64_u32 v[94:95], s[22:23], v75, 5, v[74:75]
+	v_min3_u32 v81, v86, v84, v81
+	v_sub_u32_e32 v74, v95, v75
+	v_min3_u32 v81, v90, v88, v81
+	v_mad_u64_u32 v[74:75], s[22:23], v74, 5, v[94:95]
+	v_min3_u32 v75, v74, v92, v81
+	v_cmp_gt_u32_e32 vcc, 25, v75
+	s_cbranch_vccnz .LBB53_16
+.LBB53_11:
+	s_setprio 1
+	v_mad_u64_u32 v[72:73], s[40:41], v2, 1, v[72:73]
+	v_mad_u64_u32 v[70:71], s[42:43], v1, 1, v[70:71]
+	v_mad_u64_u32 v[68:69], s[44:45], v80, 1, v[68:69]
+	v_mad_u64_u32 v[66:67], s[46:47], v82, 1, v[66:67]
+	v_mad_u64_u32 v[64:65], s[48:49], v84, 1, v[64:65]
+	v_mad_u64_u32 v[62:63], s[50:51], v86, 1, v[62:63]
+	v_mad_u64_u32 v[60:61], s[52:53], v88, 1, v[60:61]
+	v_mad_u64_u32 v[58:59], s[54:55], v90, 1, v[58:59]
+	s_setprio 2
+	v_mad_u64_u32 v[56:57], s[40:41], v90, v2, v[56:57]
+	v_mad_u64_u32 v[54:55], s[42:43], v90, v1, v[54:55]
+	v_mad_u64_u32 v[52:53], s[44:45], v90, v80, v[52:53]
+	v_mad_u64_u32 v[50:51], s[46:47], v90, v82, v[50:51]
+	s_bcnt1_i32_b64 s56, s[40:41]
+	s_add_u32 s65, s65, s56
+	s_bcnt1_i32_b64 s56, s[42:43]
+	s_add_u32 s64, s64, s56
+	s_bcnt1_i32_b64 s56, s[44:45]
+	s_add_u32 s63, s63, s56
+	s_bcnt1_i32_b64 s56, s[46:47]
+	s_add_u32 s62, s62, s56
+	s_nop 0
+	v_mad_u64_u32 v[48:49], s[48:49], v90, v84, v[48:49]
+	v_mad_u64_u32 v[46:47], s[50:51], v90, v86, v[46:47]
+	v_mad_u64_u32 v[44:45], s[52:53], v90, v88, v[44:45]
+	v_mad_u64_u32 v[42:43], s[54:55], v90, v90, v[42:43]
+	s_bcnt1_i32_b64 s57, s[48:49]
+	s_add_u32 s61, s61, s57
+	s_bcnt1_i32_b64 s57, s[50:51]
+	s_add_u32 s60, s60, s57
+	s_bcnt1_i32_b64 s57, s[52:53]
+	s_add_u32 s59, s59, s57
+	s_bcnt1_i32_b64 s57, s[54:55]
+	s_add_u32 s58, s58, s57
+	s_nop 0
+	v_mad_u64_u32 v[40:41], s[40:41], v92, v2, v[40:41]
+	v_mad_u64_u32 v[38:39], s[42:43], v92, v1, v[38:39]
+	v_mad_u64_u32 v[36:37], s[44:45], v92, v80, v[36:37]
+	v_mad_u64_u32 v[34:35], s[46:47], v92, v82, v[34:35]
+	s_bcnt1_i32_b64 s56, s[40:41]
+	s_add_u32 s39, s39, s56
+	s_bcnt1_i32_b64 s56, s[42:43]
+	s_add_u32 s38, s38, s56
+	s_bcnt1_i32_b64 s56, s[44:45]
+	s_add_u32 s37, s37, s56
+	s_bcnt1_i32_b64 s56, s[46:47]
+	s_add_u32 s36, s36, s56
+	s_nop 0
+	v_mad_u64_u32 v[32:33], s[48:49], v92, v84, v[32:33]
+	v_mad_u64_u32 v[30:31], s[50:51], v92, v86, v[30:31]
+	v_mad_u64_u32 v[28:29], s[52:53], v92, v88, v[28:29]
+	v_mad_u64_u32 v[26:27], s[54:55], v92, v90, v[26:27]
+	s_bcnt1_i32_b64 s57, s[48:49]
+	s_add_u32 s35, s35, s57
+	s_bcnt1_i32_b64 s57, s[50:51]
+	s_add_u32 s34, s34, s57
+	s_bcnt1_i32_b64 s57, s[52:53]
+	s_add_u32 s33, s33, s57
+	s_bcnt1_i32_b64 s57, s[54:55]
+	s_add_u32 s31, s31, s57
+	s_nop 0
+	v_mad_u64_u32 v[24:25], s[40:41], v74, v2, v[24:25]
+	v_mad_u64_u32 v[22:23], s[42:43], v74, v1, v[22:23]
+	v_mad_u64_u32 v[20:21], s[44:45], v74, v80, v[20:21]
+	v_mad_u64_u32 v[18:19], s[46:47], v74, v82, v[18:19]
+	s_bcnt1_i32_b64 s56, s[40:41]
+	s_add_u32 s30, s30, s56
+	s_bcnt1_i32_b64 s56, s[42:43]
+	s_add_u32 s29, s29, s56
+	s_bcnt1_i32_b64 s56, s[44:45]
+	s_add_u32 s28, s28, s56
+	s_bcnt1_i32_b64 s56, s[46:47]
+	s_add_u32 s27, s27, s56
+	s_nop 0
+	v_mad_u64_u32 v[16:17], s[48:49], v74, v84, v[16:17]
+	v_mad_u64_u32 v[14:15], s[50:51], v74, v86, v[14:15]
+	v_mad_u64_u32 v[12:13], s[52:53], v74, v88, v[12:13]
+	v_mad_u64_u32 v[10:11], s[54:55], v74, v90, v[10:11]
+	s_bcnt1_i32_b64 s57, s[48:49]
+	s_add_u32 s26, s26, s57
+	s_bcnt1_i32_b64 s57, s[50:51]
+	s_add_u32 s25, s25, s57
+	s_bcnt1_i32_b64 s57, s[52:53]
+	s_add_u32 s24, s24, s57
+	s_bcnt1_i32_b64 s57, s[54:55]
+	s_add_u32 s8, s8, s57
+	s_setprio 0
+	v_mad_u64_u32 v[74:75], s[22:23], v3, v3, 0
+	v_mad_u64_u32 v[80:81], s[22:23], v75, 5, v[74:75]
+	v_sub_u32_e32 v1, v81, v75
+	v_lshl_add_u32 v2, v1, 2, v1
+	v_add_u32_e32 v1, v2, v80
+	v_mad_u64_u32 v[74:75], s[22:23], v1, v3, 0
+	v_mad_u64_u32 v[80:81], s[22:23], v75, 5, v[74:75]
+	v_sub_u32_e32 v74, v81, v75
+	v_mad_u64_u32 v[80:81], s[22:23], v74, 5, v[80:81]
+	v_mad_u64_u32 v[74:75], s[22:23], v80, v3, 0
+	v_mad_u64_u32 v[82:83], s[22:23], v75, 5, v[74:75]
+	v_sub_u32_e32 v74, v83, v75
+	v_mad_u64_u32 v[82:83], s[22:23], v74, 5, v[82:83]
+	v_mad_u64_u32 v[74:75], s[22:23], v82, v3, 0
+	v_mad_u64_u32 v[84:85], s[22:23], v75, 5, v[74:75]
+	v_sub_u32_e32 v74, v85, v75
+	v_mad_u64_u32 v[84:85], s[22:23], v74, 5, v[84:85]
+	v_mad_u64_u32 v[74:75], s[22:23], v84, v3, 0
+	v_mad_u64_u32 v[86:87], s[22:23], v75, 5, v[74:75]
+	v_sub_u32_e32 v74, v87, v75
+	v_mad_u64_u32 v[86:87], s[22:23], v74, 5, v[86:87]
+	v_mad_u64_u32 v[74:75], s[22:23], v86, v3, 0
+	v_mad_u64_u32 v[88:89], s[22:23], v75, 5, v[74:75]
+	v_sub_u32_e32 v74, v89, v75
+	v_mad_u64_u32 v[88:89], s[22:23], v74, 5, v[88:89]
+	v_mad_u64_u32 v[74:75], s[22:23], v88, v3, 0
+	v_mad_u64_u32 v[90:91], s[22:23], v75, 5, v[74:75]
+	v_sub_u32_e32 v74, v91, v75
+	v_mad_u64_u32 v[90:91], s[22:23], v74, 5, v[90:91]
+	v_mad_u64_u32 v[74:75], s[22:23], v90, v90, 0
+	v_mad_u64_u32 v[92:93], s[22:23], v75, 5, v[74:75]
+	v_sub_u32_e32 v74, v93, v75
+	v_mad_u64_u32 v[92:93], s[22:23], v74, 5, v[92:93]
+	v_mad_u64_u32 v[74:75], s[22:23], v92, v90, 0
+	v_min3_u32 v77, v82, v80, v1
+	v_mad_u64_u32 v[94:95], s[22:23], v75, 5, v[74:75]
+	v_min3_u32 v77, v86, v84, v77
+	v_sub_u32_e32 v74, v95, v75
+	v_min3_u32 v77, v90, v88, v77
+	v_mad_u64_u32 v[74:75], s[22:23], v74, 5, v[94:95]
+	v_min3_u32 v75, v74, v92, v77
+	v_cmp_gt_u32_e32 vcc, 25, v75
+	s_cbranch_vccnz .LBB53_19
+.LBB53_12:
+	s_setprio 1
+	v_mad_u64_u32 v[72:73], s[40:41], v3, 1, v[72:73]
+	v_mad_u64_u32 v[70:71], s[42:43], v1, 1, v[70:71]
+	v_mad_u64_u32 v[68:69], s[44:45], v80, 1, v[68:69]
+	v_mad_u64_u32 v[66:67], s[46:47], v82, 1, v[66:67]
+	v_mad_u64_u32 v[64:65], s[48:49], v84, 1, v[64:65]
+	v_mad_u64_u32 v[62:63], s[50:51], v86, 1, v[62:63]
+	v_mad_u64_u32 v[60:61], s[52:53], v88, 1, v[60:61]
+	v_mad_u64_u32 v[58:59], s[54:55], v90, 1, v[58:59]
+	s_setprio 2
+	v_mad_u64_u32 v[56:57], s[40:41], v90, v3, v[56:57]
+	v_mad_u64_u32 v[54:55], s[42:43], v90, v1, v[54:55]
+	v_mad_u64_u32 v[52:53], s[44:45], v90, v80, v[52:53]
+	v_mad_u64_u32 v[50:51], s[46:47], v90, v82, v[50:51]
+	s_bcnt1_i32_b64 s56, s[40:41]
+	s_add_u32 s65, s65, s56
+	s_bcnt1_i32_b64 s56, s[42:43]
+	s_add_u32 s64, s64, s56
+	s_bcnt1_i32_b64 s56, s[44:45]
+	s_add_u32 s63, s63, s56
+	s_bcnt1_i32_b64 s56, s[46:47]
+	s_add_u32 s62, s62, s56
+	s_nop 0
+	v_mad_u64_u32 v[48:49], s[48:49], v90, v84, v[48:49]
+	v_mad_u64_u32 v[46:47], s[50:51], v90, v86, v[46:47]
+	v_mad_u64_u32 v[44:45], s[52:53], v90, v88, v[44:45]
+	v_mad_u64_u32 v[42:43], s[54:55], v90, v90, v[42:43]
+	s_bcnt1_i32_b64 s57, s[48:49]
+	s_add_u32 s61, s61, s57
+	s_bcnt1_i32_b64 s57, s[50:51]
+	s_add_u32 s60, s60, s57
+	s_bcnt1_i32_b64 s57, s[52:53]
+	s_add_u32 s59, s59, s57
+	s_bcnt1_i32_b64 s57, s[54:55]
+	s_add_u32 s58, s58, s57
+	s_nop 0
+	v_mad_u64_u32 v[40:41], s[40:41], v92, v3, v[40:41]
+	v_mad_u64_u32 v[38:39], s[42:43], v92, v1, v[38:39]
+	v_mad_u64_u32 v[36:37], s[44:45], v92, v80, v[36:37]
+	v_mad_u64_u32 v[34:35], s[46:47], v92, v82, v[34:35]
+	s_bcnt1_i32_b64 s56, s[40:41]
+	s_add_u32 s39, s39, s56
+	s_bcnt1_i32_b64 s56, s[42:43]
+	s_add_u32 s38, s38, s56
+	s_bcnt1_i32_b64 s56, s[44:45]
+	s_add_u32 s37, s37, s56
+	s_bcnt1_i32_b64 s56, s[46:47]
+	s_add_u32 s36, s36, s56
+	s_nop 0
+	v_mad_u64_u32 v[32:33], s[48:49], v92, v84, v[32:33]
+	v_mad_u64_u32 v[30:31], s[50:51], v92, v86, v[30:31]
+	v_mad_u64_u32 v[28:29], s[52:53], v92, v88, v[28:29]
+	v_mad_u64_u32 v[26:27], s[54:55], v92, v90, v[26:27]
+	s_bcnt1_i32_b64 s57, s[48:49]
+	s_add_u32 s35, s35, s57
+	s_bcnt1_i32_b64 s57, s[50:51]
+	s_add_u32 s34, s34, s57
+	s_bcnt1_i32_b64 s57, s[52:53]
+	s_add_u32 s33, s33, s57
+	s_bcnt1_i32_b64 s57, s[54:55]
+	s_add_u32 s31, s31, s57
+	s_nop 0
+	v_mad_u64_u32 v[24:25], s[40:41], v74, v3, v[24:25]
+	v_mad_u64_u32 v[22:23], s[42:43], v74, v1, v[22:23]
+	v_mad_u64_u32 v[20:21], s[44:45], v74, v80, v[20:21]
+	v_mad_u64_u32 v[18:19], s[46:47], v74, v82, v[18:19]
+	s_bcnt1_i32_b64 s56, s[40:41]
+	s_add_u32 s30, s30, s56
+	s_bcnt1_i32_b64 s56, s[42:43]
+	s_add_u32 s29, s29, s56
+	s_bcnt1_i32_b64 s56, s[44:45]
+	s_add_u32 s28, s28, s56
+	s_bcnt1_i32_b64 s56, s[46:47]
+	s_add_u32 s27, s27, s56
+	s_nop 0
+	v_mad_u64_u32 v[16:17], s[48:49], v74, v84, v[16:17]
+	v_mad_u64_u32 v[14:15], s[50:51], v74, v86, v[14:15]
+	v_mad_u64_u32 v[12:13], s[52:53], v74, v88, v[12:13]
+	v_mad_u64_u32 v[10:11], s[54:55], v74, v90, v[10:11]
+	s_bcnt1_i32_b64 s57, s[48:49]
+	s_add_u32 s26, s26, s57
+	s_bcnt1_i32_b64 s57, s[50:51]
+	s_add_u32 s25, s25, s57
+	s_bcnt1_i32_b64 s57, s[52:53]
+	s_add_u32 s24, s24, s57
+	s_bcnt1_i32_b64 s57, s[54:55]
+	s_add_u32 s8, s8, s57
+	s_setprio 0
+	v_mad_u64_u32 v[2:3], s[22:23], v4, v4, 0
+	v_mad_u64_u32 v[74:75], s[22:23], v3, 5, v[2:3]
+	v_sub_u32_e32 v1, v75, v3
+	v_lshl_add_u32 v77, v1, 2, v1
+	v_add_u32_e32 v1, v77, v74
+	v_mad_u64_u32 v[2:3], s[22:23], v1, v4, 0
+	v_mad_u64_u32 v[74:75], s[22:23], v3, 5, v[2:3]
+	v_sub_u32_e32 v2, v75, v3
+	v_mad_u64_u32 v[2:3], s[22:23], v2, 5, v[74:75]
+	v_mad_u64_u32 v[74:75], s[22:23], v2, v4, 0
+	v_mad_u64_u32 v[80:81], s[22:23], v75, 5, v[74:75]
+	v_sub_u32_e32 v3, v81, v75
+	v_mad_u64_u32 v[80:81], s[22:23], v3, 5, v[80:81]
+	v_mad_u64_u32 v[74:75], s[22:23], v80, v4, 0
+	v_mad_u64_u32 v[82:83], s[22:23], v75, 5, v[74:75]
+	v_sub_u32_e32 v74, v83, v75
+	v_mad_u64_u32 v[82:83], s[22:23], v74, 5, v[82:83]
+	v_mad_u64_u32 v[74:75], s[22:23], v82, v4, 0
+	v_mad_u64_u32 v[84:85], s[22:23], v75, 5, v[74:75]
+	v_sub_u32_e32 v74, v85, v75
+	v_mad_u64_u32 v[84:85], s[22:23], v74, 5, v[84:85]
+	v_mad_u64_u32 v[74:75], s[22:23], v84, v4, 0
+	v_mad_u64_u32 v[86:87], s[22:23], v75, 5, v[74:75]
+	v_sub_u32_e32 v74, v87, v75
+	v_mad_u64_u32 v[86:87], s[22:23], v74, 5, v[86:87]
+	v_mad_u64_u32 v[74:75], s[22:23], v86, v4, 0
+	v_mad_u64_u32 v[88:89], s[22:23], v75, 5, v[74:75]
+	v_sub_u32_e32 v74, v89, v75
+	v_mad_u64_u32 v[88:89], s[22:23], v74, 5, v[88:89]
+	v_mad_u64_u32 v[74:75], s[22:23], v88, v88, 0
+	v_mad_u64_u32 v[90:91], s[22:23], v75, 5, v[74:75]
+	v_sub_u32_e32 v74, v91, v75
+	v_mad_u64_u32 v[90:91], s[22:23], v74, 5, v[90:91]
+	v_mad_u64_u32 v[74:75], s[22:23], v90, v88, 0
+	v_min3_u32 v3, v80, v2, v1
+	v_mad_u64_u32 v[92:93], s[22:23], v75, 5, v[74:75]
+	v_min3_u32 v3, v84, v82, v3
+	v_sub_u32_e32 v74, v93, v75
+	v_min3_u32 v3, v88, v86, v3
+	v_mad_u64_u32 v[74:75], s[22:23], v74, 5, v[92:93]
+	v_min3_u32 v3, v74, v90, v3
+	v_cmp_gt_u32_e32 vcc, 25, v3
+	s_cbranch_vccnz .LBB53_22
+.LBB53_13:
+	s_setprio 1
+	v_mad_u64_u32 v[72:73], s[40:41], v4, 1, v[72:73]
+	v_mad_u64_u32 v[70:71], s[42:43], v1, 1, v[70:71]
+	v_mad_u64_u32 v[68:69], s[44:45], v2, 1, v[68:69]
+	v_mad_u64_u32 v[66:67], s[46:47], v80, 1, v[66:67]
+	v_mad_u64_u32 v[64:65], s[48:49], v82, 1, v[64:65]
+	v_mad_u64_u32 v[62:63], s[50:51], v84, 1, v[62:63]
+	v_mad_u64_u32 v[60:61], s[52:53], v86, 1, v[60:61]
+	v_mad_u64_u32 v[58:59], s[54:55], v88, 1, v[58:59]
+	s_setprio 2
+	v_mad_u64_u32 v[56:57], s[40:41], v88, v4, v[56:57]
+	v_mad_u64_u32 v[54:55], s[42:43], v88, v1, v[54:55]
+	v_mad_u64_u32 v[52:53], s[44:45], v88, v2, v[52:53]
+	v_mad_u64_u32 v[50:51], s[46:47], v88, v80, v[50:51]
+	s_bcnt1_i32_b64 s56, s[40:41]
+	s_add_u32 s65, s65, s56
+	s_bcnt1_i32_b64 s56, s[42:43]
+	s_add_u32 s64, s64, s56
+	s_bcnt1_i32_b64 s56, s[44:45]
+	s_add_u32 s63, s63, s56
+	s_bcnt1_i32_b64 s56, s[46:47]
+	s_add_u32 s62, s62, s56
+	s_nop 0
+	v_mad_u64_u32 v[48:49], s[48:49], v88, v82, v[48:49]
+	v_mad_u64_u32 v[46:47], s[50:51], v88, v84, v[46:47]
+	v_mad_u64_u32 v[44:45], s[52:53], v88, v86, v[44:45]
+	v_mad_u64_u32 v[42:43], s[54:55], v88, v88, v[42:43]
+	s_bcnt1_i32_b64 s57, s[48:49]
+	s_add_u32 s61, s61, s57
+	s_bcnt1_i32_b64 s57, s[50:51]
+	s_add_u32 s60, s60, s57
+	s_bcnt1_i32_b64 s57, s[52:53]
+	s_add_u32 s59, s59, s57
+	s_bcnt1_i32_b64 s57, s[54:55]
+	s_add_u32 s58, s58, s57
+	s_nop 0
+	v_mad_u64_u32 v[40:41], s[40:41], v90, v4, v[40:41]
+	v_mad_u64_u32 v[38:39], s[42:43], v90, v1, v[38:39]
+	v_mad_u64_u32 v[36:37], s[44:45], v90, v2, v[36:37]
+	v_mad_u64_u32 v[34:35], s[46:47], v90, v80, v[34:35]
+	s_bcnt1_i32_b64 s56, s[40:41]
+	s_add_u32 s39, s39, s56
+	s_bcnt1_i32_b64 s56, s[42:43]
+	s_add_u32 s38, s38, s56
+	s_bcnt1_i32_b64 s56, s[44:45]
+	s_add_u32 s37, s37, s56
+	s_bcnt1_i32_b64 s56, s[46:47]
+	s_add_u32 s36, s36, s56
+	s_nop 0
+	v_mad_u64_u32 v[32:33], s[48:49], v90, v82, v[32:33]
+	v_mad_u64_u32 v[30:31], s[50:51], v90, v84, v[30:31]
+	v_mad_u64_u32 v[28:29], s[52:53], v90, v86, v[28:29]
+	v_mad_u64_u32 v[26:27], s[54:55], v90, v88, v[26:27]
+	s_bcnt1_i32_b64 s57, s[48:49]
+	s_add_u32 s35, s35, s57
+	s_bcnt1_i32_b64 s57, s[50:51]
+	s_add_u32 s34, s34, s57
+	s_bcnt1_i32_b64 s57, s[52:53]
+	s_add_u32 s33, s33, s57
+	s_bcnt1_i32_b64 s57, s[54:55]
+	s_add_u32 s31, s31, s57
+	s_nop 0
+	v_mad_u64_u32 v[24:25], s[40:41], v74, v4, v[24:25]
+	v_mad_u64_u32 v[22:23], s[42:43], v74, v1, v[22:23]
+	v_mad_u64_u32 v[20:21], s[44:45], v74, v2, v[20:21]
+	v_mad_u64_u32 v[18:19], s[46:47], v74, v80, v[18:19]
+	s_bcnt1_i32_b64 s56, s[40:41]
+	s_add_u32 s30, s30, s56
+	s_bcnt1_i32_b64 s56, s[42:43]
+	s_add_u32 s29, s29, s56
+	s_bcnt1_i32_b64 s56, s[44:45]
+	s_add_u32 s28, s28, s56
+	s_bcnt1_i32_b64 s56, s[46:47]
+	s_add_u32 s27, s27, s56
+	s_nop 0
+	v_mad_u64_u32 v[16:17], s[48:49], v74, v82, v[16:17]
+	v_mad_u64_u32 v[14:15], s[50:51], v74, v84, v[14:15]
+	v_mad_u64_u32 v[12:13], s[52:53], v74, v86, v[12:13]
+	v_mad_u64_u32 v[10:11], s[54:55], v74, v88, v[10:11]
+	s_bcnt1_i32_b64 s57, s[48:49]
+	s_add_u32 s26, s26, s57
+	s_bcnt1_i32_b64 s57, s[50:51]
+	s_add_u32 s25, s25, s57
+	s_bcnt1_i32_b64 s57, s[52:53]
+	s_add_u32 s24, s24, s57
+	s_bcnt1_i32_b64 s57, s[54:55]
+	s_add_u32 s8, s8, s57
+	s_setprio 0
+	v_mad_u64_u32 v[2:3], s[22:23], v5, v5, 0
+	v_mad_u64_u32 v[74:75], s[22:23], v3, 5, v[2:3]
+	v_sub_u32_e32 v1, v75, v3
+	v_lshl_add_u32 v4, v1, 2, v1
+	v_add_u32_e32 v1, v4, v74
+	v_mad_u64_u32 v[2:3], s[22:23], v1, v5, 0
+	v_mad_u64_u32 v[74:75], s[22:23], v3, 5, v[2:3]
+	v_sub_u32_e32 v2, v75, v3
+	v_mad_u64_u32 v[2:3], s[22:23], v2, 5, v[74:75]
+	v_mad_u64_u32 v[74:75], s[22:23], v2, v5, 0
+	v_mad_u64_u32 v[80:81], s[22:23], v75, 5, v[74:75]
+	v_sub_u32_e32 v3, v81, v75
+	v_mad_u64_u32 v[80:81], s[22:23], v3, 5, v[80:81]
+	v_mad_u64_u32 v[74:75], s[22:23], v80, v5, 0
+	v_mad_u64_u32 v[82:83], s[22:23], v75, 5, v[74:75]
+	v_sub_u32_e32 v74, v83, v75
+	v_mad_u64_u32 v[82:83], s[22:23], v74, 5, v[82:83]
+	v_mad_u64_u32 v[74:75], s[22:23], v82, v5, 0
+	v_mad_u64_u32 v[84:85], s[22:23], v75, 5, v[74:75]
+	v_sub_u32_e32 v74, v85, v75
+	v_mad_u64_u32 v[84:85], s[22:23], v74, 5, v[84:85]
+	v_mad_u64_u32 v[74:75], s[22:23], v84, v5, 0
+	v_mad_u64_u32 v[86:87], s[22:23], v75, 5, v[74:75]
+	v_sub_u32_e32 v74, v87, v75
+	v_mad_u64_u32 v[86:87], s[22:23], v74, 5, v[86:87]
+	v_mad_u64_u32 v[74:75], s[22:23], v86, v5, 0
+	v_mad_u64_u32 v[88:89], s[22:23], v75, 5, v[74:75]
+	v_sub_u32_e32 v74, v89, v75
+	v_mad_u64_u32 v[88:89], s[22:23], v74, 5, v[88:89]
+	v_mad_u64_u32 v[74:75], s[22:23], v88, v88, 0
+	v_mad_u64_u32 v[90:91], s[22:23], v75, 5, v[74:75]
+	v_sub_u32_e32 v74, v91, v75
+	v_mad_u64_u32 v[92:93], s[22:23], v74, 5, v[90:91]
+	v_mad_u64_u32 v[74:75], s[22:23], v92, v88, 0
+	v_min3_u32 v3, v80, v2, v1
+	v_mad_u64_u32 v[90:91], s[22:23], v75, 5, v[74:75]
+	v_min3_u32 v3, v84, v82, v3
+	v_sub_u32_e32 v74, v91, v75
+	v_min3_u32 v3, v88, v86, v3
+	v_mad_u64_u32 v[90:91], s[22:23], v74, 5, v[90:91]
+	v_min3_u32 v3, v90, v92, v3
+	v_cmp_gt_u32_e32 vcc, 25, v3
+	s_cbranch_vccnz .LBB53_25
+.LBB53_14:
+	s_setprio 1
+	v_mad_u64_u32 v[72:73], s[40:41], v5, 1, v[72:73]
+	v_mad_u64_u32 v[70:71], s[42:43], v1, 1, v[70:71]
+	v_mad_u64_u32 v[68:69], s[44:45], v2, 1, v[68:69]
+	v_mad_u64_u32 v[66:67], s[46:47], v80, 1, v[66:67]
+	v_mad_u64_u32 v[64:65], s[48:49], v82, 1, v[64:65]
+	v_mad_u64_u32 v[62:63], s[50:51], v84, 1, v[62:63]
+	v_mad_u64_u32 v[60:61], s[52:53], v86, 1, v[60:61]
+	v_mad_u64_u32 v[58:59], s[54:55], v88, 1, v[58:59]
+	s_setprio 2
+	v_mad_u64_u32 v[56:57], s[40:41], v88, v5, v[56:57]
+	v_mad_u64_u32 v[54:55], s[42:43], v88, v1, v[54:55]
+	v_mad_u64_u32 v[52:53], s[44:45], v88, v2, v[52:53]
+	v_mad_u64_u32 v[50:51], s[46:47], v88, v80, v[50:51]
+	s_bcnt1_i32_b64 s56, s[40:41]
+	s_add_u32 s65, s65, s56
+	s_bcnt1_i32_b64 s56, s[42:43]
+	s_add_u32 s64, s64, s56
+	s_bcnt1_i32_b64 s56, s[44:45]
+	s_add_u32 s63, s63, s56
+	s_bcnt1_i32_b64 s56, s[46:47]
+	s_add_u32 s62, s62, s56
+	s_nop 0
+	v_mad_u64_u32 v[48:49], s[48:49], v88, v82, v[48:49]
+	v_mad_u64_u32 v[46:47], s[50:51], v88, v84, v[46:47]
+	v_mad_u64_u32 v[44:45], s[52:53], v88, v86, v[44:45]
+	v_mad_u64_u32 v[42:43], s[54:55], v88, v88, v[42:43]
+	s_bcnt1_i32_b64 s57, s[48:49]
+	s_add_u32 s61, s61, s57
+	s_bcnt1_i32_b64 s57, s[50:51]
+	s_add_u32 s60, s60, s57
+	s_bcnt1_i32_b64 s57, s[52:53]
+	s_add_u32 s59, s59, s57
+	s_bcnt1_i32_b64 s57, s[54:55]
+	s_add_u32 s58, s58, s57
+	s_nop 0
+	v_mad_u64_u32 v[40:41], s[40:41], v92, v5, v[40:41]
+	v_mad_u64_u32 v[38:39], s[42:43], v92, v1, v[38:39]
+	v_mad_u64_u32 v[36:37], s[44:45], v92, v2, v[36:37]
+	v_mad_u64_u32 v[34:35], s[46:47], v92, v80, v[34:35]
+	s_bcnt1_i32_b64 s56, s[40:41]
+	s_add_u32 s39, s39, s56
+	s_bcnt1_i32_b64 s56, s[42:43]
+	s_add_u32 s38, s38, s56
+	s_bcnt1_i32_b64 s56, s[44:45]
+	s_add_u32 s37, s37, s56
+	s_bcnt1_i32_b64 s56, s[46:47]
+	s_add_u32 s36, s36, s56
+	s_nop 0
+	v_mad_u64_u32 v[32:33], s[48:49], v92, v82, v[32:33]
+	v_mad_u64_u32 v[30:31], s[50:51], v92, v84, v[30:31]
+	v_mad_u64_u32 v[28:29], s[52:53], v92, v86, v[28:29]
+	v_mad_u64_u32 v[26:27], s[54:55], v92, v88, v[26:27]
+	s_bcnt1_i32_b64 s57, s[48:49]
+	s_add_u32 s35, s35, s57
+	s_bcnt1_i32_b64 s57, s[50:51]
+	s_add_u32 s34, s34, s57
+	s_bcnt1_i32_b64 s57, s[52:53]
+	s_add_u32 s33, s33, s57
+	s_bcnt1_i32_b64 s57, s[54:55]
+	s_add_u32 s31, s31, s57
+	s_nop 0
+	v_mad_u64_u32 v[24:25], s[40:41], v90, v5, v[24:25]
+	v_mad_u64_u32 v[22:23], s[42:43], v90, v1, v[22:23]
+	v_mad_u64_u32 v[20:21], s[44:45], v90, v2, v[20:21]
+	v_mad_u64_u32 v[18:19], s[46:47], v90, v80, v[18:19]
+	s_bcnt1_i32_b64 s56, s[40:41]
+	s_add_u32 s30, s30, s56
+	s_bcnt1_i32_b64 s56, s[42:43]
+	s_add_u32 s29, s29, s56
+	s_bcnt1_i32_b64 s56, s[44:45]
+	s_add_u32 s28, s28, s56
+	s_bcnt1_i32_b64 s56, s[46:47]
+	s_add_u32 s27, s27, s56
+	s_nop 0
+	v_mad_u64_u32 v[16:17], s[48:49], v90, v82, v[16:17]
+	v_mad_u64_u32 v[14:15], s[50:51], v90, v84, v[14:15]
+	v_mad_u64_u32 v[12:13], s[52:53], v90, v86, v[12:13]
+	v_mad_u64_u32 v[10:11], s[54:55], v90, v88, v[10:11]
+	s_bcnt1_i32_b64 s57, s[48:49]
+	s_add_u32 s26, s26, s57
+	s_bcnt1_i32_b64 s57, s[50:51]
+	s_add_u32 s25, s25, s57
+	s_bcnt1_i32_b64 s57, s[52:53]
+	s_add_u32 s24, s24, s57
+	s_bcnt1_i32_b64 s57, s[54:55]
+	s_add_u32 s8, s8, s57
+	s_setprio 0
+	s_add_i32 s69, s69, -1
+	s_cmp_eq_u32 s69, 0
+	v_lshl_add_u64 v[78:79], v[78:79], 0, s[18:19]
+	s_cbranch_scc1 .LBB53_29
+	s_waitcnt vmcnt(0)
+	v_mov_b32_e32 v5, v9
+	v_mov_b32_e32 v4, v8
+	v_mov_b32_e32 v3, v7
+	v_mov_b32_e32 v2, v6
+	s_branch .LBB53_10
diff --git a/sidekick_amd/csrc/bsgs.h b/sidekick_amd/csrc/bsgs.h
--- a/sidekick_amd/csrc/bsgs.h
+++ b/sidekick_amd/csrc/bsgs.h
@@ -216,6 +216,98 @@
     return r;
 }
 
+#define QK_LP(D, DH, Y, X)                                                                             \
+    "v_mad_u64_u32 v[" #D ":" #DH "], s[58:59], " Y ", " X ", 0\n\t"                                   \
+    "v_mad_u64_u32 v[6:7], s[58:59], v" #DH ", 5, v[" #D ":" #DH "]\n\t"                               \
+    "v_mad_u64_u32 v[" #D ":" #DH "], s[58:59], v7, 5, v[" #D ":" #DH "]\n\t"
+#define QK_BT1 QK_LP(8, 9, "v28", "%[id]")
+#define QK_BT2 QK_LP(28, 29, "v30", "%[id]") QK_BT1
+#define QK_BT3 QK_LP(30, 31, "v32", "%[id]") QK_BT2
+#define QK_BT4 QK_LP(32, 33, "v34", "%[id]") QK_BT3
+#define QK_BT5 QK_LP(34, 35, "v36", "%[id]") QK_BT4
+#define QK_BT6 QK_LP(36, 37, "v38", "%[id]") QK_BT5
+#define QK_BABIES4 QK_LP(30, 31, "%[id]", "%[id]") QK_BT2
+#define QK_BABIES6 QK_LP(34, 35, "%[id]", "%[id]") QK_BT4
+#define QK_BABIES8 QK_LP(38, 39, "%[id]", "%[id]") QK_BT6
+#define QK_BMIN4 "v_min3_u32 v9, v30, v28, v8\n\t"
+#define QK_BMIN6 QK_BMIN4 "v_min3_u32 v9, v9, v34, v32\n\t"
+#define QK_BMIN8 QK_BMIN6 "v_min3_u32 v9, v9, v38, v36\n\t"
+#define QK_BOUT4 "=&{v30}"(B[1]), "=&{v28}"(B[2]), "=&{v8}"(B[3])
+#define QK_BOUT6 "=&{v34}"(B[1]), "=&{v32}"(B[2]), "=&{v30}"(B[3]), "=&{v28}"(B[4]), "=&{v8}"(B[5])
+#define QK_BOUT8                                                                                       \
+    "=&{v38}"(B[1]), "=&{v36}"(B[2]), "=&{v34}"(B[3]), "=&{v32}"(B[4]), "=&{v30}"(B[5]), "=&{v28}"(B[6]), \
+        "=&{v8}"(B[7])
+#define QK_BCLOB4 "v31", "v29"
+#define QK_BCLOB6 QK_BCLOB4, "v35", "v33"
+#define QK_BCLOB8 QK_BCLOB6, "v39", "v37"
+#define QK_GIANTS0
+#define QK_GIANTS1 QK_LP(10, 11, "v8", "v8")
+#define QK_GIANTS2 QK_GIANTS1 QK_LP(12, 13, "v10", "v8")
+#define QK_GIANTS3 QK_GIANTS2 QK_LP(14, 15, "v12", "v8")
+#define QK_GIANTS4 QK_GIANTS3 QK_LP(16, 17, "v14", "v8")
+#define QK_GIANTS5 QK_GIANTS4 QK_LP(18, 19, "v16", "v8")
+#define QK_GIANTS6 QK_GIANTS5 QK_LP(20, 21, "v18", "v8")
+#define QK_GIANTS7 QK_GIANTS6 QK_LP(22, 23, "v20", "v8")
+#define QK_GIANTS8 QK_GIANTS7 QK_LP(24, 25, "v22", "v8")
+#define QK_GIANTS9 QK_GIANTS8 QK_LP(26, 27, "v24", "v8")
+#define QK_GMIN0
+#define QK_GMIN1 "v_min_u32_e32 v9, v9, v10\n\t"
+#define QK_GMIN2 "v_min3_u32 v9, v9, v10, v12\n\t"
+#define QK_GMIN3 QK_GMIN2 "v_min_u32_e32 v9, v9, v14\n\t"
+#define QK_GMIN4 QK_GMIN2 "v_min3_u32 v9, v9, v14, v16\n\t"
+#define QK_GMIN5 QK_GMIN4 "v_min_u32_e32 v9, v9, v18\n\t"
+#define QK_GMIN6 QK_GMIN4 "v_min3_u32 v9, v9, v18, v20\n\t"
+#define QK_GMIN7 QK_GMIN6 "v_min_u32_e32 v9, v9, v22\n\t"
+#define QK_GMIN8 QK_GMIN6 "v_min3_u32 v9, v9, v22, v24\n\t"
+#define QK_GMIN9 QK_GMIN8 "v_min_u32_e32 v9, v9, v26\n\t"
+#define QK_GOUT0
+#define QK_GOUT1 , "=&{v10}"(G[0])
+#define QK_GOUT2 QK_GOUT1, "=&{v12}"(G[1])
+#define QK_GOUT3 QK_GOUT2, "=&{v14}"(G[2])
+#define QK_GOUT4 QK_GOUT3, "=&{v16}"(G[3])
+#define QK_GOUT5 QK_GOUT4, "=&{v18}"(G[4])
+#define QK_GOUT6 QK_GOUT5, "=&{v20}"(G[5])
+#define QK_GOUT7 QK_GOUT6, "=&{v22}"(G[6])
+#define QK_GOUT8 QK_GOUT7, "=&{v24}"(G[7])
+#define QK_GOUT9 QK_GOUT8, "=&{v26}"(G[8])
+#define QK_GCLOB0
+#define QK_GCLOB1 , "v11"
+#define QK_GCLOB2 QK_GCLOB1, "v13"
+#define QK_GCLOB3 QK_GCLOB2, "v15"
+#define QK_GCLOB4 QK_GCLOB3, "v17"
+#define QK_GCLOB5 QK_GCLOB4, "v19"
+#define QK_GCLOB6 QK_GCLOB5, "v21"
+#define QK_GCLOB7 QK_GCLOB6, "v23"
+#define QK_GCLOB8 QK_GCLOB7, "v25"
+#define QK_GCLOB9 QK_GCLOB8, "v27"
+
+template <int NB, int NG>
+struct LazyChain {
+    static constexpr bool fused = false;
+};
+#define QK_CHAIN(NB, NG)                                                                               \
+    template <>                                                                                        \
+    struct LazyChain<NB, NG> {                                                                         \
+        static constexpr bool fused = true;                                                            \
+        static __device__ __forceinline__ uint32_t run(uint32_t id, uint32_t (&B)[NB],                 \
+                                                       uint32_t (&G)[NG ? NG : 1]) {                   \
+            uint32_t mn;                                                                               \
+            (void)G;                                                                                   \
+            asm(QK_BABIES##NB QK_GIANTS##NG QK_BMIN##NB QK_GMIN##NG                                    \
+                : "=&{v9}"(mn), QK_BOUT##NB QK_GOUT##NG                                                \
+                : [id] "v"(id)                                                                         \
+                : "v6", "v7", QK_BCLOB##NB QK_GCLOB##NG, "s58", "s59");                                \
+            return mn;                                                                                 \
+        }                                                                                              \
+    };
+#define QK_CHAINS(NB)                                                                                  \
+    QK_CHAIN(NB, 0) QK_CHAIN(NB, 1) QK_CHAIN(NB, 2) QK_CHAIN(NB, 3) QK_CHAIN(NB, 4) QK_CHAIN(NB, 5)    \
+    QK_CHAIN(NB, 6) QK_CHAIN(NB, 7) QK_CHAIN(NB, 8) QK_CHAIN(NB, 9)
+QK_CHAINS(4)
+QK_CHAINS(6)
+QK_CHAINS(8)
+
+constexpr uint32_t WRAP_BELOW = 25u;
 template <class C>
 __device__ __forceinline__ uint32_t powers(uint32_t id, uint32_t (&B)[C::NB], uint32_t (&A)[C::ROWS],
                                            uint32_t base = 0, uint32_t xb = 0, uint32_t *xnext = nullptr) {
@@ -223,15 +315,20 @@
     B[0] = id;
     if constexpr (C::OFF) {
         uint32_t mn = 0xFFFFFFFFu;
-#pragma unroll
-        for (int b = 1; b < NB; ++b) B[b] = mulfold32_min(B[b - 1], B[0], mn);
+        if constexpr (LazyChain<NB, 0>::fused) {
+            uint32_t G[1];
+            mn = LazyChain<NB, 0>::run(id, B, G);
+        } else {
+#pragma unroll
+            for (int b = 1; b < NB; ++b) B[b] = mulfold32_min(B[b - 1], B[0], mn);
+        }
         const uint32_t xn = B[NB - 1];
         if constexpr (C::XC & 1) A[0] = xb;
         else A[0] = pow_uniform(xn, base / NB, [&](uint32_t u, uint32_t v) { return mulfold32_min(u, v, mn); });
 #pragma unroll
         for (int a = 1; a < NA; ++a) A[a] = mulfold32_min(A[a - 1], xn, mn);
         if constexpr ((C::XC & 2) != 0) *xnext = mulfold32_min(A[NA - 1], xn, mn);
-        return mn < 25u;
+        return mn;
     } else if constexpr (C::FOLD == 0) {
         uint32_t wrapped = 0;
 #pragma unroll
@@ -239,8 +336,18 @@
         A[0] = B[NB - 1];
 #pragma unroll
         for (int a = 1; a < NA - 1; ++a) A[a] = mulfold32_fast(A[a - 1], A[0], wrapped);
-        return wrapped;
+        return wrapped ? 0u : 0xFFFFFFFFu;
     } else {
+        constexpr int NG = NA - 2 + ((C::XC & 2) != 0 ? 1 : 0);
+        if constexpr (!C::TREE && LazyChain<NB, NG>::fused) {
+            uint32_t G[NG ? NG : 1];
+            const uint32_t mn = LazyChain<NB, NG>::run(id, B, G);
+            A[0] = B[NB - 1];
+#pragma unroll
+            for (int a = 1; a < NA - 1; ++a) A[a] = G[a - 1];
+            if constexpr ((C::XC & 2) != 0) *xnext = G[NA - 2];
+            return mn;
+        }
         uint32_t mn = 0xFFFFFFFFu;
         if constexpr (C::TREE) {
 #pragma unroll
@@ -257,7 +364,7 @@
 #pragma unroll
         for (int a = 1; a < NA - 1; ++a) A[a] = mulfold32_min(A[a - 1], A[0], mn);
         if constexpr ((C::XC & 2) != 0) *xnext = mulfold32_min(A[NA - 2], A[0], mn);
-        return mn < 25u;
+        return mn;
     }
 }
 template <class C>
@@ -366,11 +473,13 @@
 __device__ __forceinline__ void one(Acc<C::NB, C::NA, C::ROWS> &S, uint32_t id, uint32_t base = 0, uint32_t xb = 0,
                                     uint32_t *xnext = nullptr) {
     uint32_t B[C::NB], A[C::ROWS];
-    const uint32_t w = powers<C>(id, B, A, base, xb, xnext);
+    const uint32_t mn = powers<C>(id, B, A, base, xb, xnext);
+    prio_enter<C>();
+    if constexpr (C::PRIO != 0) __builtin_amdgcn_sched_barrier(0);
+    const bool w = mn < WRAP_BELOW;
     if (__builtin_expect(__any(w), 0)) {
         if (w) powers_exact<C>(B, A, base, xb, xnext);
     }
-    prio_enter<C>();
     accumulate<C>(S, B, A);
     prio_exit<C>();
 }
@@ -379,8 +488,8 @@
 __device__ __forceinline__ void two(Acc<C::NB, C::NA, C::ROWS> &S, uint32_t id0, uint32_t id1) {
     static_assert(!C::OFF, "pairs: plain passes only");
     uint32_t B0[C::NB], A0[C::ROWS], B1[C::NB], A1[C::ROWS];
-    const uint32_t w0 = powers<C>(id0, B0, A0);
-    const uint32_t w1 = powers<C>(id1, B1, A1);
+    const bool w0 = powers<C>(id0, B0, A0) < WRAP_BELOW;
+    const bool w1 = powers<C>(id1, B1, A1) < WRAP_BELOW;
     if (__builtin_expect(__any(w0 | w1), 0)) {
         if (w0) powers_exact<C>(B0, A0);
         if (w1) powers_exact<C>(B1, A1);
@@ -408,10 +517,11 @@
 }
 
 template <class C, class Out>
-__device__ __forceinline__ void finish(const Acc<C::NB, C::NA, C::ROWS> &S, uint32_t T, Out out) {
+__device__ __forceinline__ void finish(const Acc<C::NB, C::NA, C::ROWS> &S, uint32_t T, Out out,
+                                       uint32_t tid = threadIdx.x) {
     constexpr int NB = C::NB, NA = C::NA;
     __shared__ uint64_t sm[WAVES * NB * NA];
-    const int lane = threadIdx.x & 63, wave = threadIdx.x >> 6;
+    const int lane = tid & 63, wave = tid >> 6;
 #pragma unroll
     for (int a = 0; a < NA; ++a) {
 #pragma unroll
@@ -435,7 +545,7 @@
         }
     }
     __syncthreads();
-    for (uint32_t m = threadIdx.x; m < T; m += BLOCK) {
+    for (uint32_t m = tid; m < T; m += BLOCK) {
         uint64_t s = 0;
 #pragma unroll
         for (int w = 0; w < WAVES; ++w) s += sm[w * (NB * NA) + m];
@@ -463,6 +573,10 @@
     constexpr bool XI = (C::XC & 1) != 0, XO = (C::XC & 2) != 0;
     Acc<C::NB, C::NA, C::ROWS> S;
     clear<C>(S);
+    const uint64_t gbase64 = gtid - threadIdx.x;
+    const uint32_t gb_lo = (uint32_t)__builtin_amdgcn_readfirstlane((int)(uint32_t)gbase64);
+    const uint32_t gb_hi = (uint32_t)__builtin_amdgcn_readfirstlane((int)(uint32_t)(gbase64 >> 32));
+    const uint32_t wave_s = (uint32_t)__builtin_amdgcn_readfirstlane((int)(threadIdx.x >> 6));
     const uint64_t h = head < n ? head : n;
     const uint64_t nbody = (n - h) >> 2;
     const uint4 *__restrict__ v = reinterpret_cast<const uint4 *>(ids + h);
@@ -472,8 +586,9 @@
     const uint4 *__restrict__ p = v + gtid;
     const uint4 *pc = XI ? reinterpret_cast<const uint4 *>(xin + h) + gtid : nullptr;
     uint4 *po = XO ? reinterpret_cast<uint4 *>(xout + h) + gtid : nullptr;
+    const uint4 *const vend = v + nbody;
     uint4 nxt = make_uint4(0, 0, 0, 0), nxc = make_uint4(0, 0, 0, 0), xo = make_uint4(0, 0, 0, 0);
-    if (iters) {
+    if (p < vend) {
         nxt = *p;
         if constexpr (XI) nxc = *pc;
     }
@@ -494,20 +609,24 @@
     }
     for (; it < tmax; ++it) {
         const uint4 w = nxt, c = nxc;
+        const bool cur = p < vend;
         p += nthr;
         nxt = make_uint4(0, 0, 0, 0);
-        if (it + 1 < iters) nxt = *p;
+        if (p < vend) nxt = *p;
         if constexpr (XI) {
             pc += nthr;
-            if (it + 1 < iters) nxc = *pc;
+            if (p < vend) nxc = *pc;
         }
         four<C>(S, w, base, c, &xo);
         if constexpr (XO) {
-            if (it < iters) *po = xo;
+            if (cur) *po = xo;
             po += nthr;
         }
+        (void)cur;
     }
     const uint64_t tail0 = h + (nbody << 2);
+    const uint32_t tid = wave_s * 64u + __lane_id();
+    gtid = (((uint64_t)gb_hi << 32) | gb_lo) + tid;
     {
         const bool in = gtid < h;
         uint32_t xn = 0;
@@ -521,7 +640,7 @@
         if (XO && in) xout[tail0 + gtid] = xn;
     }
 
-    finish<C>(S, T, out);
+    finish<C>(S, T, out, tid);
 }
 
 template <class C>
diff --git a/sidekick_amd/csrc/field.h b/sidekick_amd/csrc/field.h
--- a/sidekick_amd/csrc/field.h
+++ b/sidekick_amd/csrc/field.h
@@ -60,19 +60,27 @@
     const uint64_t P = (uint64_t)y * x;
     const uint32_t Ph = (uint32_t)(P >> 32);
     const uint64_t Q = P + (uint64_t)Ph * C32;
-    const uint32_t tl = (uint32_t)Q, th = (uint32_t)(Q >> 32) - Ph;
-    const uint32_t m = th * C32;
-    uint32_t r = tl + m;
+    const uint32_t Qh = (uint32_t)(Q >> 32);
+    const uint32_t m = (Qh - Ph) * C32;
+    uint32_t r = (uint32_t)P + C32 * Qh;
     if (r < m) r += C32;
     return r;
 }
 
 QK_HD uint32_t mulfold32_min(uint32_t y, uint32_t x, uint32_t &mn) {
+#if defined(__HIP_DEVICE_COMPILE__)
+    uint64_t R = (uint64_t)y * x;
+    asm("v_mad_u64_u32 v[6:7], s[58:59], %1, 5, %0\n\t"
+        "v_mad_u64_u32 %0, s[58:59], v7, 5, %0"
+        : "+v"(R)
+        : "v"((uint32_t)(R >> 32))
+        : "v6", "v7", "s58", "s59");
+    const uint32_t r = (uint32_t)R;
+#else
     const uint64_t P = (uint64_t)y * x;
-    const uint32_t Ph = (uint32_t)(P >> 32);
-    const uint64_t Q = P + (uint64_t)Ph * C32;
-    const uint32_t tl = (uint32_t)Q, th = (uint32_t)(Q >> 32) - Ph;
-    const uint32_t r = tl + th * C32;
+    const uint64_t Q = P + (uint64_t)(uint32_t)(P >> 32) * C32;
+    const uint32_t r = (uint32_t)P + C32 * (uint32_t)(Q >> 32);
+#endif
     mn = r < mn ? r : mn;
     return r;
 }
diff --git a/sidekick_amd/csrc/packets.hip b/sidekick_amd/csrc/packets.hip
--- a/sidekick_amd/csrc/packets.hip
+++ b/sidekick_amd/csrc/packets.hip
@@ -98,7 +98,7 @@
         if constexpr (SH) {
             using Pw = typename C::Pw;
             uint32_t B[8], A[Pw::ROWS];
-            const uint32_t w = bsgs::powers<Pw>(cls == 1 ? id : 0u, B, A);
+            const bool w = bsgs::powers<Pw>(cls == 1 ? id : 0u, B, A) < bsgs::WRAP_BELOW;
             if (__builtin_expect(__any(w), 0)) {
                 if (w) bsgs::powers_exact<Pw>(B, A);
             }
```
